# rgcgithub/regenie

Hardware: NVIDIA H100
Metric: step1_level0_snps_per_sec (higher is better)
Workload: dtype int8 Gram + int8 prediction (both exact integer sums) + tf32x3 factorisation + f64 refinement / statistics

## Files before the change

regenie_b200/csrc/bed_kernels.cu:

```cuda
#include "kernels.cuh"

namespace rg {

__device__ __forceinline__ uint32_t plink_to_code(uint32_t v, int ref_first) {
  const uint32_t lut = ref_first ? 0x9Cu : 0x1Eu;
  return (lut >> (2 * v)) & 3u;
}

__global__ void bed_relayout_kernel(const uint8_t* __restrict__ packed, int64_t row_stride, int bs,
                                    const int32_t* __restrict__ file_idx_pad, const int32_t* __restrict__ word_base,
                                    const uint32_t* __restrict__ word_keep, int ref_first,
                                    uint32_t* __restrict__ gp, int64_t words_per_row) {
  const int64_t w = blockIdx.x * (int64_t)blockDim.x + threadIdx.x;
  const int row = blockIdx.y;
  if (w >= words_per_row) return;
  uint32_t out = 0;
  const int base = (row < bs) ? __ldg(word_base + w) : -1;
  if (base >= 0) {
    const uint8_t* p = packed + (int64_t)row * row_stride + (base >> 2);
    const int64_t left = row_stride - (base >> 2);
    uint64_t x = 0;
#pragma unroll
    for (int b = 0; b < 5; ++b)
      if (b < left) x |= (uint64_t)__ldg(p + b) << (8 * b);
    const uint32_t v = (uint32_t)(x >> (2 * (base & 3)));
    const uint32_t H = (v >> 1) & 0x55555555u, Lo = v & 0x55555555u;
    const uint32_t oh = ref_first ? Lo : (~H & 0x55555555u);
    out = ((oh << 1) | (H ^ Lo)) & __ldg(word_keep + w);
  } else if (base == -2) {
    const uint8_t* prow = packed + (int64_t)row * row_stride;
    const int4* fi4 = reinterpret_cast<const int4*>(file_idx_pad + w * 16);
#pragma unroll
    for (int q = 0; q < 4; ++q) {
      const int4 f = __ldg(fi4 + q);
      const int fi[4] = {f.x, f.y, f.z, f.w};
#pragma unroll
      for (int k = 0; k < 4; ++k) {
        uint32_t code = 0;
        if (fi[k] >= 0) {
          const uint32_t b = __ldg(prow + (fi[k] >> 2));
          code = plink_to_code((b >> (2 * (fi[k] & 3))) & 3u, ref_first);
        }
        out |= code << (2 * (q * 4 + k));
      }
    }
  }
  gp[(int64_t)row * words_per_row + w] = out;
}

__device__ __forceinline__ uint32_t spread_sel(uint32_t b) {
  return (b & 0x3u) | ((b & 0xCu) << 2) | ((b & 0x30u) << 4) | ((b & 0xC0u) << 6);
}

__global__ void bed_expand_fp8_kernel(const uint32_t* __restrict__ gp, int64_t words_per_row,
                                      int rows_p, uint8_t* __restrict__ z, int64_t npad) {
  const int64_t w = blockIdx.x * (int64_t)blockDim.x + threadIdx.x;
  const int row = blockIdx.y;
  if (w >= words_per_row) return;
  const uint32_t word = __ldg(gp + (int64_t)row * words_per_row + w);
  const uint32_t kLutG = 0x00100800u;
  const uint32_t kLutM = 0x08000000u;
  uint4 g, m;
  uint32_t* gv = reinterpret_cast<uint32_t*>(&g);
  uint32_t* mv = reinterpret_cast<uint32_t*>(&m);
#pragma unroll
  for (int k = 0; k < 4; ++k) {
    const uint32_t sel = spread_sel((word >> (8 * k)) & 0xFFu);
    gv[k] = __byte_perm(kLutG, 0, sel);
    mv[k] = __byte_perm(kLutM, 0, sel);
  }
  *reinterpret_cast<uint4*>(z + (int64_t)row * npad + w * 16) = g;
  *reinterpret_cast<uint4*>(z + (int64_t)(rows_p + row) * npad + w * 16) = m;
}

void launch_bed_relayout(const uint8_t* packed, int64_t row_stride, int bs, int rows_p,
                         const int32_t* file_idx_pad, const int32_t* word_base, const uint32_t* word_keep, int ref_first,
                         uint32_t* gp, int64_t npad,
                         cudaStream_t s) {
  const int64_t wpr = npad / 16;
  dim3 grid((unsigned)ceil_div(wpr, 256), rows_p);
  bed_relayout_kernel<<<grid, 256, 0, s>>>(packed, row_stride, bs, file_idx_pad, word_base, word_keep, ref_first, gp, wpr);
}

void launch_bed_expand_fp8(const uint32_t* gp, int rows_p, uint8_t* z, int64_t npad, cudaStream_t s) {
  const int64_t wpr = npad / 16;
  dim3 grid((unsigned)ceil_div(wpr, 256), rows_p);
  bed_expand_fp8_kernel<<<grid, 256, 0, s>>>(gp, wpr, rows_p, z, npad);
}

}
```

regenie_b200/csrc/context.cuh:

```cuda
#pragma once
#include <map>
#include <memory>

#include "../../include/rg_b200.h"
#include "kernels.cuh"

struct rg_ctx;
namespace rg { void ensure_W(::rg_ctx* h); }

struct rg_ctx {
  int kind = 0;
  int device = 0;
  cudaStream_t stream = nullptr;
  int64_t launches = 0;

  int64_t N = 0, Npad = 0, n_analyzed = 0;
  int C = 0, P = 0, K = 1, R = 0, R1 = 0, loocv = 0;
  int bs_max = 0, rows_p_max = 0, total_blocks = 0, cpp = 0;
  int64_t B = 0;

  std::vector<int64_t> fold_sizes, fold_pad_start, fold_pad_len;
  std::vector<int32_t> pad_of;
  std::vector<int32_t> src_of;
  std::vector<uint8_t> in_analysis;
  std::vector<int32_t> cached_sample_idx;
  bool file_idx_valid = false;
  int nchunks = 0;

  rg::DevBuf<double> xy;
  rg::DevBuf<uint8_t> mask;
  rg::DevBuf<uint8_t> is_real;
  rg::DevBuf<int32_t> tile_fold;
  rg::DevBuf<int4> chunks;
  rg::DevBuf<int2> fold_chunks;
  rg::DevBuf<int2> fold_k;
  rg::DevBuf<double> XtX_f, XtY_f, lambda, neff;
  rg::DevBuf<int32_t> file_idx_pad;
  rg::DevBuf<int32_t> word_base;
  rg::DevBuf<uint32_t> word_keep;
  rg::DevBuf<unsigned long long> err_slot;
  cudaStream_t poll_stream = nullptr;
  unsigned long long* poll_host = nullptr;

  struct Lane {
    cudaStream_t stream = nullptr;
    cudaEvent_t done = nullptr;
    cudaEvent_t h2d_done = nullptr;
    bool h2d_recorded = false;
    rg::DevBuf<uint8_t> packed_dev;
    rg::DevBuf<uint8_t> packed_buf[2];
    cudaStream_t copy_stream = nullptr;
    cudaEvent_t relayout_done[2] = {nullptr, nullptr};
    bool relayout_recorded[2] = {false, false};
    int packed_flip = 0;
    rg::DevBuf<uint8_t> pgen_in;
    rg::DevBuf<uint32_t> gp;
    rg::DevBuf<uint8_t> z;
    rg::DevBuf<float> zz;
    rg::DevBuf<unsigned long long> miss_total;
    rg::DevBuf<int2> miss_seg;
    rg::DevBuf<int32_t> miss_list;
    rg::DevBuf<uint32_t> gt;
    rg::DevBuf<float> tstat;
    rg::DevBuf<int32_t> cnt_part, cnt_fold;
    rg::DevBuf<double> sum_part, sum_fold;
    rg::DevBuf<double> mu, inv_sd, Bv, Af, Qf, gty_f, rhs;
    rg::DevBuf<double> cm;
    rg::DevBuf<double> inv;
    rg::DevBuf<double> gam, gmu, cvec, part, mean_invsd;
    std::map<int, CUtensorMap> tmaps;
    rg::DevBuf<uint8_t> dig;
    rg::DevBuf<double> wraw;
    rg::DevBuf<double*> wraw_tab;
    rg::DevBuf<double> dscale;
    std::map<int, CUtensorMap> dmaps;
    std::map<int, CUtensorMap> gmaps;
    rg::DevBuf<uint8_t> dense_in;
    rg::DevBuf<double> gd, dpart, dpart_y;
    std::unique_ptr<rg::MixedSolver> mx;
    rg::DevBuf<double> mx_Af, mx_b, mx_x, mx_r;
    rg::DevBuf<unsigned int> mx_fail;
    unsigned int* mx_fail_host = nullptr;
    cudaEvent_t mx_ev = nullptr;
    bool mx_pending = false;
    int mx_bs = 0, mx_block_id = 0;
    int last_pred_i8 = 0, last_mx_n = 0;
    bool last_gram_dense = false;
  };
  std::vector<std::unique_ptr<Lane>> lanes;
  int next_lane = 0, last_lane = 0;
  rg::DevBuf<uint8_t> packed_dev;
  rg::DevBuf<uint32_t> gp;
  struct TileList {
    rg::DevBuf<int2> buf;
    int count = 0;
  };
  std::map<int, TileList> tile_lists, stat_tile_lists;
  bool stats_tc = false;
  int stat_drows = 0;
  rg::DevBuf<uint8_t> xyD;
  rg::DevBuf<double> xy_scale;
  CUtensorMap tmD;

  rg::DevBuf<double> W;
  int last_bs = 0, last_rows_p = 0, last_nC = 0, last_n_aug = 0, last_nmat = 0;

  rg::DevBuf<int4> l1_chunks;
  rg::DevBuf<int2> l1_fold_chunks;
  int l1_nchunks = 0;
  rg::DevBuf<double> l1_part, l1_part_y, l1_cm, l1_inv, l1_beta, l1_sums, l1_part_out, l1_tau, l1_pred;
  rg::DevBuf<int32_t> l1_chr_cols;
  rg::DevBuf<double> l1_zrows, l1_hvec, l1_bvec;
  std::vector<int32_t> best_idx;
  std::vector<double> prs_host;
  int l1_nC = 0;
  int l1_nmat = 0, l1_n_aug = 0;
  int64_t l1_chunk_len = 0;
  bool l1_done = false;
  rg::DevBuf<double*> W_tab;
  std::vector<double*> W_host_tab;
  std::vector<uint8_t> W_owned;
  std::vector<void*> W_peer_mapped;
  std::vector<uint8_t> l1_select;
  bool l1_bt = false;
  rg::DevBuf<double> lg_Ws, lg_eta, lg_p, lg_wm, lg_res, lg_off, lg_beta, lg_score, lg_q, lg_devp, lg_scal;
  rg::DevBuf<int8_t> lg_ym;
  rg::DevBuf<int2> lg_all_chunks;

  int strict = 0, dp = 0;
  std::vector<double> Xh;
  std::vector<uint8_t> maskh;
  rg::DevBuf<double> F, s2_part, s2_sums, s2_maskcount, s2_YtX, s2_XmX, s2_scf;
  rg::DevBuf<double> s2_out_d;
  rg::DevBuf<int32_t> s2_out_i;
  double* s2_hd = nullptr;
  int32_t* s2_hi = nullptr;
  size_t s2_host_cap = 0;
  bool s2_tc = false;
  int s2_drows = 0, s2_nchunk = 0, s2_ncol = 0;
  int64_t s2_chunk_len = 0;
  rg::DevBuf<uint8_t> s2_z3, s2_FD;
  rg::DevBuf<double> s2_Fscale;
  rg::DevBuf<float> s2_T;
  rg::DevBuf<int2> s2_fold_k;
  std::map<int, std::unique_ptr<rg::DevBuf<int2>>> s2_tile_lists;
  rg::DevBuf<uint8_t> s2_ones;
  CUtensorMap s2_tmD;
  std::map<int, CUtensorMap> s2_tmZ;
  std::map<int, int> s2_ntiles;
  std::vector<uint8_t> s2_male;
  int s2_col_male = -1, bt_col_male = -1;
  rg::DevBuf<uint8_t> s2_nonpar;
  bool s2_nonpar_set = false;
  rg::DevBuf<double> s2_male_tot;
  int bt_mode = 0, bt_dp = 0, bt_ncol = 0;
  int s2_fcols = 0;
  bool s2_chr_set = false, bt_chr_set = false;
  int s2_last_bs = 0;
  int s2_sums_rows = 0, bt_sums_rows = 0, bt_sums_dp = 0;
  static constexpr int kStageSlots = 4;
  rg::DevBuf<uint8_t> s2_stage[kStageSlots];
  cudaStream_t s2_copy_stream = nullptr;
  cudaEvent_t s2_stage_ev[kStageSlots] = {nullptr, nullptr, nullptr, nullptr};
  bool s2_stage_pending[kStageSlots] = {false, false, false, false};
  rg::DevBuf<uint8_t> probs_dev, miss_dev;
  rg::DevBuf<uint8_t> inflate_comp, inflate_raw;
  rg::DevBuf<uint64_t> inflate_offs;
  rg::DevBuf<int32_t> inflate_status;
  rg::DevBuf<uint8_t> pgen_in, pgen_rows;
  rg::DevBuf<unsigned long long> pgen_err;
  rg::DevBuf<uint32_t> dz;
  rg::DevBuf<double> bt_F, bt_w, bt_gs, bt_xw, bt_off, bt_coltot, bt_xwy, bt_part, bt_sums, bt_nnz, bt_n510;
  rg::DevBuf<double> bt_xtwg, bt_mu, bt_info, firth_gvec, firth_out, bt_den, bt_phat;
  rg::DevBuf<int8_t> bt_ym, firth_cflag;
  rg::DevBuf<int2> bt_cnt_part;
  rg::DevBuf<int32_t> firth_sel, firth_status;

  bool gram_dense = false;
  int64_t miss_cap = 0;

  int solver_mixed = 1;
  float mx_tol = 1e-9f;
  int64_t mx_blocks = 0, mx_fallbacks = 0;

  bool timing = false;
  cudaEvent_t ev0 = nullptr, ev1 = nullptr;
  std::map<std::string, std::pair<double, int64_t>> timers;
  std::vector<std::tuple<std::string, cudaEvent_t, cudaEvent_t>> pending;
};

namespace rg {
void require_gpu(int device);
void ensure_file_idx(rg_ctx* h, const int32_t* sample_idx);
void flush_timers(rg_ctx* h);
void sync_lanes(rg_ctx* h);
void pgen_check_errors(rg_ctx* h);
}

#define RG_API_BEGIN try {
#define RG_API_END                         \
  }                                        \
  catch (const rg::Error& e) {             \
    rg::set_last_error(e.msg);             \
    return 1;                              \
  }                                        \
  catch (const std::exception& e) {        \
    rg::set_last_error(e.what());          \
    return 1;                              \
  }                                        \
  return 0;
```

regenie_b200/csrc/gram_wgmma.cu:

```cuda
#include "kernels.cuh"
#include "wgmma_sm90.cuh"

namespace rg {

namespace {

using namespace sm90;

constexpr int BM = 128;
constexpr int BK = 128;
constexpr int STAGES = 4;
constexpr int A_BYTES = BM * BK;
constexpr int NTHREADS = 288;

}

template <int BN>
__global__ void __launch_bounds__(NTHREADS, 1)
gram_s8_wgmma_kernel(const __grid_constant__ CUtensorMap tmZ, const __grid_constant__ CUtensorMap tmB,
                      const int2* __restrict__ tiles,
                      const int2* __restrict__ fold_k, float* __restrict__ out, int ldo,
                      int64_t fold_stride, float out_scale, const unsigned long long* __restrict__ miss_total,
                      unsigned long long miss_cap, int miss_tile0) {
  constexpr int B_BYTES = BN * BK;
  constexpr int STAGE_BYTES = A_BYTES + B_BYTES;
  constexpr int NACC = BN / 2;
  extern __shared__ uint8_t smem_raw[];
  const uint32_t raw = smem_u32(smem_raw);
  const uint32_t base = (raw + 1023u) & ~1023u;
  uint8_t* gen_base = smem_raw + (base - raw);
  const uint32_t sA = base;
  const uint32_t sB = base + STAGES * A_BYTES;
  uint64_t* bars = reinterpret_cast<uint64_t*>(gen_base + STAGES * STAGE_BYTES);
  const uint32_t full_bar = smem_u32(bars);
  const uint32_t empty_bar = smem_u32(bars + STAGES);

  const int warp = __shfl_sync(0xffffffffu, threadIdx.x >> 5, 0), lane = threadIdx.x & 31;
  const int2 tile = tiles[blockIdx.x];
  if (miss_total && tile.x >= miss_tile0 && *miss_total <= miss_cap) return;
  const int2 fk = fold_k[blockIdx.y];
  const int nkb = fk.y;

  if (warp == 8 && lane == 0) {
    for (int s = 0; s < STAGES; ++s) {
      mbar_init(full_bar + 8 * s, 1);
      mbar_init(empty_bar + 8 * s, 2);
    }
    fence_barrier_init();
    prefetch_tmap(&tmZ);
    prefetch_tmap(&tmB);
  }
  __syncthreads();

  if (warp == 8) {
    if (lane == 0) {
      for (int kb = 0; kb < nkb; ++kb) {
        const int s = kb % STAGES;
        const uint32_t ph = (kb / STAGES) & 1;
        mbar_wait(empty_bar + 8 * s, ph ^ 1);
        mbar_expect_tx(full_bar + 8 * s, STAGE_BYTES);
        const int kc = (fk.x + kb) * BK;
        tma_load_2d(sA + s * A_BYTES, &tmZ, full_bar + 8 * s, kc, tile.x * BM);
        tma_load_2d(sB + s * B_BYTES, &tmB, full_bar + 8 * s, kc, tile.y * BN);
        if (BN == 256) tma_load_2d(sB + s * B_BYTES + A_BYTES, &tmB, full_bar + 8 * s, kc, tile.y * BN + 128);
      }
    }
    return;
  }

  const int wg = warp >> 2;
  int32_t acc[NACC];
#pragma unroll
  for (int i = 0; i < NACC; ++i) acc[i] = 0;
  fence_regs(acc);
  for (int kb = 0; kb < nkb; ++kb) {
    const int s = kb % STAGES;
    const uint32_t ph = (kb / STAGES) & 1;
    mbar_wait(full_bar + 8 * s, ph);
    const uint64_t da = desc_k128(sA + s * A_BYTES + wg * (64 * BK));
    const uint64_t db = desc_k128(sB + s * B_BYTES);
    wgmma_fence();
#pragma unroll
    for (int k = 0; k < BK / 32; ++k) {
      if constexpr (BN == 256) wgmma_s8_n256(acc, da + (uint64_t)(2 * k), db + (uint64_t)(2 * k));
      else wgmma_s8_n128(acc, da + (uint64_t)(2 * k), db + (uint64_t)(2 * k));
    }
    wgmma_commit();
    wgmma_wait<1>();
    if (kb > 0 && (warp & 3) == 0 && lane == 0) mbar_arrive(empty_bar + 8 * ((kb - 1) % STAGES));
  }
  wgmma_wait<0>();
  fence_regs(acc);

  const int r0 = tile.x * BM + wg * 64 + (warp & 3) * 16 + (lane >> 2);
  float* obase = out + (int64_t)blockIdx.y * fold_stride + tile.y * BN + 2 * (lane & 3);
#pragma unroll
  for (int j = 0; j < BN / 8; ++j) {
    *reinterpret_cast<float2*>(obase + (int64_t)r0 * ldo + 8 * j) =
        make_float2((float)acc[4 * j] * out_scale, (float)acc[4 * j + 1] * out_scale);
    *reinterpret_cast<float2*>(obase + (int64_t)(r0 + 8) * ldo + 8 * j) =
        make_float2((float)acc[4 * j + 2] * out_scale, (float)acc[4 * j + 3] * out_scale);
  }
}

__global__ void gram_reference_kernel(const uint8_t* __restrict__ z, int64_t npad, int rows2, int k0, int k1,
                                      float* __restrict__ out, int ldo) {
  const int j = blockIdx.x * blockDim.x + threadIdx.x;
  const int i = blockIdx.y;
  if (j >= rows2 || j > i) return;
  const uint8_t* zi = z + (int64_t)i * npad;
  const uint8_t* zj = z + (int64_t)j * npad;
  int acc = 0;
  for (int t = k0; t < k1; ++t) {
    const int a = zi[t] >> 3;
    const int b = zj[t] >> 3;
    acc += a * b;
  }
  out[(int64_t)i * ldo + j] = (float)acc;
}

typedef CUresult (*EncodeTiledFn)(CUtensorMap*, CUtensorMapDataType, cuuint32_t, void*, const cuuint64_t*,
                                  const cuuint64_t*, const cuuint32_t*, const cuuint32_t*, CUtensorMapInterleave,
                                  CUtensorMapSwizzle, CUtensorMapL2promotion, CUtensorMapFloatOOBfill);

static EncodeTiledFn get_encode_fn() {
  static EncodeTiledFn fn = nullptr;
  if (!fn) {
    void* p = nullptr;
    cudaDriverEntryPointQueryResult qres;
    RG_CUDA(cudaGetDriverEntryPoint("cuTensorMapEncodeTiled", &p, cudaEnableDefault, &qres));
    RG_CHECK(p != nullptr && qres == cudaDriverEntryPointSuccess, "cuTensorMapEncodeTiled not available");
    fn = reinterpret_cast<EncodeTiledFn>(p);
  }
  return fn;
}

void make_gram_tensor_map(CUtensorMap* tm, const uint8_t* z, int64_t npad, int rows2) {
  const cuuint64_t gdim[2] = {(cuuint64_t)npad, (cuuint64_t)rows2};
  const cuuint64_t gstride[1] = {(cuuint64_t)npad};
  const cuuint32_t box[2] = {BK, 128};
  const cuuint32_t estr[2] = {1, 1};
  CUresult r = get_encode_fn()(tm, CU_TENSOR_MAP_DATA_TYPE_UINT8, 2, const_cast<uint8_t*>(z), gdim, gstride, box,
                               estr, CU_TENSOR_MAP_INTERLEAVE_NONE, CU_TENSOR_MAP_SWIZZLE_128B,
                               CU_TENSOR_MAP_L2_PROMOTION_L2_256B, CU_TENSOR_MAP_FLOAT_OOB_FILL_NONE);
  RG_CHECK(r == CUDA_SUCCESS, "cuTensorMapEncodeTiled failed (" + std::to_string((int)r) + ")");
}

size_t gram_smem_bytes(int bn) {
  return (size_t)STAGES * (A_BYTES + bn * BK) + 1024 + 128;
}

void gram_tile_list(int rows2, std::vector<int2>& tiles) {
  tiles.clear();
  for (int nj = 0; nj < rows2 / 256; ++nj)
    for (int mi = 2 * nj; mi < rows2 / BM; ++mi) tiles.push_back(make_int2(mi, nj));
}

void launch_gram_wgmma(const CUtensorMap& tm, const CUtensorMap& tmB, const int2* tiles, int ntiles, const int2* fold_k, int K,
                         float* out, int ldo, int64_t fold_stride, float out_scale, cudaStream_t s, int bn,
                         const unsigned long long* miss_total, int64_t miss_cap, int miss_tile0) {
  RG_CHECK(bn == 256 || bn == 128, "gram tiles are 128 x 256 or 128 x 128");
  dim3 grid(ntiles, K);
  if (bn == 256) {
    ensure_dyn_smem(reinterpret_cast<const void*>(gram_s8_wgmma_kernel<256>), gram_smem_bytes(256));
    gram_s8_wgmma_kernel<256><<<grid, NTHREADS, gram_smem_bytes(256), s>>>(tm, tmB, tiles, fold_k, out, ldo, fold_stride, out_scale,
                                                                                     miss_total, miss_cap, miss_tile0);
  } else {
    ensure_dyn_smem(reinterpret_cast<const void*>(gram_s8_wgmma_kernel<128>), gram_smem_bytes(128));
    gram_s8_wgmma_kernel<128><<<grid, NTHREADS, gram_smem_bytes(128), s>>>(tm, tmB, tiles, fold_k, out, ldo, fold_stride, out_scale,
                                                                                     miss_total, miss_cap, miss_tile0);
  }
}

void launch_gram_reference(const uint8_t* z, int64_t npad, int rows2, int k0, int k1, float* out, int ldo,
                           cudaStream_t s) {
  dim3 grid((unsigned)ceil_div(rows2, 128), rows2);
  gram_reference_kernel<<<grid, 128, 0, s>>>(z, npad, rows2, k0, k1, out, ldo);
}

}
```

regenie_b200/csrc/kernels.cuh:

```cuda
#pragma once
#include "common.cuh"

namespace rg {

constexpr int kMaxFolds = 16;
constexpr int kMaxCov = 64;
constexpr int kMaxRidge = 8;
constexpr int kMaxPhenoTile = 8;
constexpr int kLimbs = 9;
constexpr int kLimbsI8 = 5;
constexpr int kLimbQI8 = 50;

void launch_bed_relayout(const uint8_t* packed, int64_t row_stride, int bs, int rows_p,
                         const int32_t* file_idx_pad, const int32_t* word_base, const uint32_t* word_keep, int ref_first,
                         uint32_t* gp, int64_t npad,
                         cudaStream_t s);
void launch_bed_expand_fp8(const uint32_t* gp, int rows_p, uint8_t* z, int64_t npad, cudaStream_t s);

struct SnpFinalizeArgs {
  int bs, rows_p, C, P, K, cpp, loocv;
  long long n_analyzed;
  double numtol;
  const int32_t* cnt_fold;
  const double* sum_fold;
  const double* XtX_f;
  const double* XtY_f;
  double *mu, *inv_sd;
  double* Bv;
  double *Af, *Qf;
  double *gty_f, *rhs;
  unsigned long long* err_slot;
  long long err_base;
};

struct AssembleArgs {
  int bs, rows_p, nC, C, K, R, loocv;
  const float* zz;
  int64_t ldz, zz_fold_stride;
  const double *mu, *inv_sd, *Bv, *Af, *Qf;
  const double* lambda;
  double* cm;
  int64_t cm_stride;
  int ldc;
  float* planes = nullptr;
  float* lplanes = nullptr;
};

void launch_l0_stats(const uint32_t* gp, int64_t npad, const double* xy, int cpp, const int4* chunks,
                     int nchunks, int rows_p, int32_t* cnt_part, double* sum_part, cudaStream_t s);
void launch_l0_fold_reduce(const int32_t* cnt_part, const double* sum_part, int rows_p, int cpp,
                           const int2* fold_chunks, int K, int32_t* cnt_fold, double* sum_fold,
                           cudaStream_t s);
void launch_l0_snp_finalize(const SnpFinalizeArgs& a, cudaStream_t s);
void launch_l0_assemble(const AssembleArgs& a, const double* rhs, int P, int Ppad, int nmat, cudaStream_t s);

void make_gram_tensor_map(CUtensorMap* tm, const uint8_t* z, int64_t npad, int rows2);
size_t gram_smem_bytes(int bn = 256);
constexpr int kStatQ = 14;
constexpr int kStatOnesRow = 126;
void launch_l0_xy_digits(const double* xy, int cpp, int ncol, int64_t npad, const uint8_t* is_real, double* scale,
                         uint8_t* D, cudaStream_t s);
void launch_l0_stats_finish(const float* T, int ldt, int64_t t_fold_stride, const float* zz, int ldz,
                            int64_t zz_fold_stride, int rows_p, int cpp, int ncol, int K, const double* scale,
                            int32_t* cnt_fold, double* sum_fold, cudaStream_t s);
void gram_tile_list(int rows2, std::vector<int2>& tiles);
void launch_gram_wgmma(const CUtensorMap& tm, const CUtensorMap& tmB, const int2* tiles, int ntiles, const int2* fold_k, int K,
                         float* out, int ldo, int64_t fold_stride, float out_scale, cudaStream_t s, int bn = 256,
                         const unsigned long long* miss_total = nullptr, int64_t miss_cap = 0, int miss_tile0 = 0);
constexpr float kZScaleGram = 1.f / 64;
constexpr float kZScaleStat = 1.f / 8;
constexpr double kMissSparseRate = 0.015;
void launch_miss_list(const uint32_t* gp, int64_t npad, int rows_p, const int2* fold_k, int K, unsigned long long* total,
                      int64_t cap, int2* seg, int32_t* list, cudaStream_t s);
void launch_miss_transpose(const uint32_t* gp, int64_t npad, int rows_p, const unsigned long long* total, int64_t cap,
                           uint32_t* gt, cudaStream_t s);
void launch_miss_sparse(const uint32_t* gt, int rows_p, const int2* seg, const int32_t* list, int K,
                        const unsigned long long* total, int64_t cap, float* zz, int64_t fold_stride, cudaStream_t s);
void launch_gram_reference(const uint8_t* z, int64_t npad, int rows2, int k0, int k1, float* out, int ldo,
                           cudaStream_t s);

void launch_chol_factor(double* cm, int64_t stride, int nC, int n_aug, int batch, double* inv,
                        unsigned long long* err_slot, long long err_base, cudaStream_t s);
void launch_chol_backsolve(double* cm, int64_t stride, int nC, int P, int batch, const double* inv,
                           cudaStream_t s);
int chol_num_launches(int nC);
size_t chol_inv_elems(int nC, int batch);
void launch_chol_rows_backsolve(double* cm, int64_t stride, int nC, int row0, int nrows, int batch,
                                const double* inv, cudaStream_t s);

struct Tf32GemmEpilogue {
  int n;
  int64_t out_mat_stride;
  float* out;
  int mirror;
  int b_cols_local;
  int negate;
  int lower_only;
  const double* cin;
  int64_t cin_mat_stride;
  int cin_ld, cin_mat_div;
  const double* diag_add;
  int diag_mod;
  int c_chunks;
  int c_mat_div;
};
void make_tf32_operand_tensor_map(CUtensorMap* tm, const float* base, int cols, int rows, int batch);
void make_f32_rows_tensor_map(CUtensorMap* tm, const float* base, int cols, int64_t rows, int box_cols, int box_rows);
void launch_tf32x3_gemm(const CUtensorMap& tmA, const CUtensorMap& tmB, const int4* tiles, int ntiles, int batch,
                        const Tf32GemmEpilogue& ep, cudaStream_t s, const CUtensorMap* tmC = nullptr);

constexpr int kMxMaxSteps = 6;
class MixedSolver {
 public:
  MixedSolver();
  ~MixedSolver();
  MixedSolver(const MixedSolver&) = delete;
  MixedSolver& operator=(const MixedSolver&) = delete;
  static int dim_for(int bs);
  void prepare(int n, int K, int R, int Pp);
  float* a_planes();
  float* l_planes();
  void solve(const double* Af, const double* lambda, const double* bvec, double* xvec, double* rvec, int P, int steps,
             float tol, unsigned int* fail_flag, cudaStream_t s, bool first_col_ready = false);
  static int launches_per_solve(int n, int steps, int P);
  const float* debug_planes(int which) const;
 private:
  struct Impl;
  Impl* impl;
};
void launch_l0_assemble_sym(const AssembleArgs& a, const double* rhs, int P, int Pp, double* bvec, cudaStream_t s);

void launch_dense_from_dosage(const uint8_t* probs, const uint8_t* miss, int64_t n_file, int bs, const int32_t* file_idx_pad,
                              int ref_first, double* gd, int64_t npad, cudaStream_t s);
void launch_dense_from_f64(const double* G, int64_t n_file, int bs, const int32_t* file_idx_pad, double* gd, int64_t npad,
                           cudaStream_t s);
void launch_dense_prepare(double* gd, int64_t npad, int bs, const int32_t* file_idx_pad, const double* xy, int cpp, int C,
                          long long n_analyzed, double numtol, double* mu, double* sd, unsigned long long* err_slot,
                          long long err_base, cudaStream_t s);
void launch_dense_assemble(const double* part, int64_t part_stride, int ldp, const double* part_y, int64_t part_y_stride,
                           const int2* fold_chunks, int K, int R, const double* lambda, int bs, int nC, int P, double* cm,
                           int64_t cm_stride, int loocv, cudaStream_t s);
void launch_dense_loocv_fill(const double* gd, int64_t npad, int bs, int nC, double* cm, int64_t cm_stride, int row0, int R,
                             cudaStream_t s);
void launch_dense_predict(const double* gd, int64_t npad, int bs, const double* cm, int64_t cm_stride, int ldc, int nC, int R,
                          int P, const int32_t* tile_fold, const uint8_t* mask, double* const* W, int col0, cudaStream_t s);

struct PredictArgs {
  int bs, rows_p, C, P, R, Qp, cpp, col0;
  int64_t npad, words_per_row;
  const uint32_t* gp;
  const int32_t* tile_fold;
  const double *gam, *gmu;
  const double* cvec;
  const double* xy;
  const uint8_t* mask;
  double* const* W;
  double* part;
};
void launch_l0_gamma(const double* cm, int64_t cm_stride, int ldc, int nC, int R, int P, int Qp,
                     int bs, int rows_p, int K, const double* mu, const double* inv_sd,
                     const double* Bv, int C, double* gam, double* gmu, double* cvec, cudaStream_t s);
void launch_l0_predict(const PredictArgs& a, int ntiles, cudaStream_t s);
void launch_l0_standardize(const double* part, int ntiles, int Qp, int Q, int P, const double* neff,
                           double* mean_invsd, double* const* W, int64_t npad, int col0,
                           const uint8_t* is_real, cudaStream_t s, const double* const* src = nullptr, int src_col0 = 0);
int predict_qt();

struct PredictTcArgs {
  int rows_p, C, P, Q, Qp, cpp, col0, ngroups;
  int64_t npad;
  const int32_t* tile_fold;
  const double* scale;
  const double* cvec;
  const double* xy;
  const uint8_t* mask;
  double* const* W;
  double* part;
};
void make_byte_tensor_map(CUtensorMap* tm, const uint8_t* basep, int64_t inner, int64_t rows);
void make_gp_tensor_map(CUtensorMap* tm, const uint32_t* gp, int64_t words_per_row, int64_t rows);
int launch_l0_colsum(double* const* W, int64_t npad, int col0, int P, int Q, int Qp, double* part,
                     cudaStream_t s);
size_t predict_i8_dig_bytes(int K, int ngroups, int rows_p);
void launch_l0_coef_i8(const double* cm, int64_t cm_stride, int ldc, int nC, int R, int P, int Q, int Qp, int bs,
                       int rows_p, int K, const double* mu, const double* inv_sd, const double* Bv, int C, double* gam,
                       double* gmu, double* cvec, double* scale, uint8_t* dig, int ngroups, cudaStream_t s);
void launch_l0_predict_i8(const CUtensorMap& tmG, const CUtensorMap& tmD, const PredictTcArgs& a, int ntiles,
                          cudaStream_t s);

void launch_l1_gram(const double* W, int64_t ldw, int B, const int4* chunks, int nchunks, double* part,
                    int64_t part_stride, int ldp, cudaStream_t s);
void launch_l1_xty(const double* W, int64_t ldw, const double* xy, int cpp, int ycol, const int4* chunks,
                   int nchunks, double* part_y, int B, cudaStream_t s);
void launch_l1_assemble(const double* part, int64_t part_stride, int ldp, const double* part_y,
                        const int2* fold_chunks, int K, int R1, const double* tau, int B, int nC, double* cm,
                        int64_t cm_stride, int loocv, cudaStream_t s);
void launch_l1_pred_sums(const double* W, int64_t ldw, int B, int R1, const double* beta, int ldb,
                         const int32_t* tile_fold, const double* xy, int cpp, int ycol, double* part_out,
                         int ntiles, double* out, cudaStream_t s);
void launch_l1_chr_pred(const double* W, int64_t ldw, int nchr, const int32_t* chr_col_start, const double* beta,
                        int ldb, int R1, int best, const int32_t* tile_fold, double* pred, int64_t npad,
                        cudaStream_t s);

void launch_l0_loocv_fill(const uint32_t* gp, int64_t npad, int bs, int nC, const double* mu, const double* inv_sd,
                          const double* Bv, int C, const double* xy, int cpp, double* cm, int64_t cm_stride,
                          int nrow0, int R, cudaStream_t s);
void launch_l0_loocv_pred(const double* cm, int64_t cm_stride, int nC, int bs, int Ppad, int P, int R,
                          const double* xy, int cpp, int C, const uint8_t* mask, int64_t npad, double* const* W,
                          int col0, double* part, int Qp, cudaStream_t s);
void launch_l0_loocv_std_apply(double* const* W, int64_t npad, int col0, int P, int Q, const uint8_t* mask,
                               const double* mean_invsd, cudaStream_t s);
void launch_l1_loocv_fill(const double* W, int64_t ldw, int B, int nC, double* cm, int64_t cm_stride, int nrow0,
                          int R1, int64_t npad, cudaStream_t s);
void launch_l1_loocv_sums(const double* cm, int64_t cm_stride, int nC, int B, int nrow0, const double* xy, int cpp,
                          int ycol, double* part, int R1, int ntiles, double* out, cudaStream_t s);
void launch_rows_sqnorm(const double* rows, int nC, int B, double* out, int ntiles, cudaStream_t s);

void launch_l1_scale_rows(const double* W, int64_t ldw, int B, const double* wm, double* Ws, cudaStream_t s);
void launch_l1_bt_eta(const double* W, int64_t ldw, int B, const double* beta, const double* offset, const int8_t* ym,
                      double* eta, double* pv, double* wm, double* resid, double* dev_part, double* dev_out,
                      cudaStream_t s);
void launch_l1_bt_score(const double* part_y, int nchunks, int B, int nC, double tau, const double* beta, double* score,
                        double* rhs_row, cudaStream_t s);
void launch_l1_bt_loo_sums(const double* eta, const double* q, const double* wm, const double* resid, const int8_t* ym,
                           double eps, double* fvec, double* part, double* out6, int64_t npad, cudaStream_t s);
void launch_l1_bt_chr_pred(const double* W, int64_t ldw, int nC, const double* zrows, const double* fvec,
                           const double* bvec, int nchr, const int32_t* chr_col_start, double* pred, int64_t npad,
                           cudaStream_t s);
void launch_l1_loocv_chr_pred(const double* W, int64_t ldw, int B, int nC, const double* zrows, const double* hvec,
                              const double* bvec, const double* xy, int cpp, int ycol, int nchr,
                              const int32_t* chr_col_start, double* pred, int64_t npad, cudaStream_t s);
void launch_l0_std_reduce_only(const double* part, int ntiles, int Qp, int Q, int P, const double* neff,
                               double* mean_invsd, cudaStream_t s);

struct S2FinalizeArgs {
  int bs, C, P, dp, strict;
  long long n_analyzed, n_samples;
  double min_mac, numtol;
  const double* sums;
  const double* mask_count;
  const double* YtX;
  const double* XmX;
  const double* scf_sv;
  const uint8_t* non_par = nullptr;
  int col_male = -1;
  const double* male_tot = nullptr;
  const double* nz_count = nullptr;
  const double* info_sums = nullptr;
  double* info = nullptr;
  double *af, *mac, *af_all, *mac_all, *scale_fac, *stat, *beta, *se, *chisq;
  int32_t *ns, *ns_all, *flags;
};
void launch_s2_stats(const uint32_t* gp, int64_t npad, const double* F, int dp, const int4* chunks, int nchunks,
                     int rows_p, double* part, double* sums, cudaStream_t s);
void launch_s2_finalize(const S2FinalizeArgs& a, cudaStream_t s);
void launch_bed_expand3_fp8(const uint32_t* gp, int rows_p, uint8_t* z, int64_t npad, cudaStream_t s);
void launch_s2_bt_bed_finish(const float* T, int ldt, int64_t chunk_stride, int nchunk, int rows_p, int dp, int D,
                             const double* scale, double* sums4, double* nnz, double* n2, cudaStream_t s);
void launch_gp_to_dz(const uint32_t* gp, int rows_p, uint32_t* dz, int64_t npad, cudaStream_t s);
void launch_s2_stats_finish(const float* T, int ldt, int64_t chunk_stride, int nchunk, int rows_p, int dp, int D,
                            const double* scale, double* sums, cudaStream_t s);

struct S2BtFinalizeArgs {
  int bs, C, P, dp, with_flip;
  long long n_analyzed, n_samples;
  double min_mac, numtol;
  const double* sums;
  const double* col_tot;
  const double* xwy;
  const uint8_t* non_par = nullptr;
  int col_male = -1;
  double unit = 255.0;
  const double* nz_count;
  const double* n510;
  double *af, *mac, *info, *af_all, *mac_all, *scale_fac, *stat, *beta, *se, *chisq, *xtwg, *mu, *den;
  int32_t *ns, *ns_all, *flags;
};
void launch_dosage_relayout(const uint8_t* probs, const uint8_t* miss, int64_t n_file, int bs, int rows_p,
                            const int32_t* file_idx_pad, int ref_first, uint32_t* dz, int64_t npad, cudaStream_t s);
void launch_dosage_stats(const uint32_t* dz, int64_t npad, const double* F, int dp, const int4* chunks, int nchunks,
                         int rows_p, double* part, int2* part_cnt, double* sums, double* nnz, double* n510, cudaStream_t s,
                         int ncol = 0 );
void launch_s2_bt_finalize(const S2BtFinalizeArgs& a, cudaStream_t s);
void launch_dosage_scale(const double* sums4, int rows_p, int dp, double* sums3, double* se, cudaStream_t s);

struct FirthArgs {
  int n_sel, C, P, dp, niter;
  double tol, maxstep;
  int64_t npad;
  const int32_t *sel_var, *sel_trait;
  const uint32_t* dz;
  const double* F;
  const double *w, *gs, *xw, *off;
  const int8_t* ym;
  const double* xtwg;
  const double* mu;
  const double* mac;
  const int32_t* flags;
  double* gvec;
  int8_t* cflag;
  double *beta, *se, *lrt;
  int32_t* status;
};
void launch_s2_firth(const FirthArgs& a, cudaStream_t s);

struct SpaArgs {
  int n_sel, C, P, dp, niter;
  double tol;
  int64_t npad;
  const int32_t *sel_var, *sel_trait;
  const uint32_t* dz;
  const double* F;
  const double *w, *gs, *xw, *phat;
  const int8_t* ym;
  const double* xtwg;
  const double* mu;
  const double *stat, *den;
  const int32_t* flags;
  double* gvec;
  int8_t* cflag;
  double* pval;
  int32_t* status;
};
void launch_s2_spa(const SpaArgs& a, cudaStream_t s);

}
```

regenie_b200/csrc/rg_api.cu:

```cuda
#include <string.h>

#include <algorithm>
#include <mutex>

#include "context.cuh"

namespace rg {

static thread_local std::string g_last_error;
void set_last_error(const std::string& m) { g_last_error = m; }

bool is_device_pointer(const void* p) {
  cudaPointerAttributes at;
  cudaError_t e = cudaPointerGetAttributes(&at, p);
  if (e != cudaSuccess) {
    cudaGetLastError();
    return false;
  }
  return at.type == cudaMemoryTypeDevice || at.type == cudaMemoryTypeManaged;
}

void copy_to_device(void* dst, const void* src, size_t bytes, cudaStream_t stream) {
  if (bytes == 0) return;
  RG_CUDA(cudaMemcpyAsync(dst, src, bytes, cudaMemcpyDefault, stream));
}

struct ScopedTimer {
  rg_ctx* h;
  std::string name;
  cudaEvent_t a = nullptr, b = nullptr;
  cudaStream_t st;
  ScopedTimer(rg_ctx* h_, const char* n, cudaStream_t s_) : h(h_), name(n), st(s_) {
    if (!h->timing) return;
    cudaEventCreate(&a);
    cudaEventCreate(&b);
    cudaEventRecord(a, st);
  }
  ~ScopedTimer() {
    if (!h->timing) return;
    cudaEventRecord(b, st);
    h->pending.emplace_back(name, a, b);
  }
};

void flush_timers(rg_ctx* h) {
  for (auto& t : h->pending) {
    float ms = 0.f;
    cudaEventSynchronize(std::get<2>(t));
    cudaEventElapsedTime(&ms, std::get<1>(t), std::get<2>(t));
    auto& acc = h->timers[std::get<0>(t)];
    acc.first += ms;
    acc.second += 1;
    cudaEventDestroy(std::get<1>(t));
    cudaEventDestroy(std::get<2>(t));
  }
  h->pending.clear();
}

void require_gpu(int device) {
  int n = 0;
  cudaError_t e = cudaGetDeviceCount(&n);
  if (e != cudaSuccess || n == 0) {
    cudaGetLastError();
    throw Error{"no CUDA device available: librg_b200 has no CPU fallback"};
  }
  RG_CHECK(device >= 0 && device < n, "invalid CUDA device ordinal");
  cudaDeviceProp prop;
  RG_CUDA(cudaGetDeviceProperties(&prop, device));
  RG_CHECK(prop.major == 9 && prop.minor == 0, std::string("librg_b200 is built for sm_90a only; device is sm_") +
                                 std::to_string(prop.major) + std::to_string(prop.minor));
}

static void build_layout(rg_ctx* h, const double* X, const double* Y, const uint8_t* mask,
                         const uint8_t* in_analysis, const int64_t* fold_sizes) {
  const int64_t N = h->N;
  const int K = h->K, C = h->C, P = h->P;
  h->fold_sizes.assign(K, 0);
  if (h->loocv) {
    h->fold_sizes[0] = N;
  } else {
    int64_t tot = 0;
    for (int f = 0; f < K; ++f) {
      RG_CHECK(fold_sizes[f] > 0, "fold sizes must be positive");
      h->fold_sizes[f] = fold_sizes[f];
      tot += fold_sizes[f];
    }
    RG_CHECK(tot == N, "fold sizes must sum to n_samples");
  }
  h->fold_pad_start.assign(K, 0);
  h->fold_pad_len.assign(K, 0);
  int64_t off = 0;
  for (int f = 0; f < K; ++f) {
    h->fold_pad_start[f] = off;
    h->fold_pad_len[f] = round_up(h->fold_sizes[f], kFoldPad);
    off += h->fold_pad_len[f];
  }
  h->Npad = off;
  RG_CHECK(h->Npad < (1ll << 31), "padded sample count must fit in int32");
  h->pad_of.assign(N, 0);
  h->src_of.assign(h->Npad, -1);
  std::vector<int32_t> tile_fold(h->Npad / 128);
  {
    int64_t s = 0;
    for (int f = 0; f < K; ++f) {
      for (int64_t o = 0; o < h->fold_sizes[f]; ++o, ++s) {
        h->pad_of[s] = (int32_t)(h->fold_pad_start[f] + o);
        h->src_of[h->fold_pad_start[f] + o] = (int32_t)s;
      }
      for (int64_t t = h->fold_pad_start[f]; t < h->fold_pad_start[f] + h->fold_pad_len[f]; t += 128)
        tile_fold[t / 128] = f;
    }
  }
  h->in_analysis.assign(in_analysis, in_analysis + N);

  h->cpp = (int)round_up(C + P, 16);
  std::vector<double> xy((size_t)h->Npad * h->cpp, 0.0);
  std::vector<uint8_t> maskp((size_t)P * h->Npad, 0), is_real(h->Npad, 0);
  h->maskh.assign(mask, mask + (size_t)N * P);
  for (int64_t s = 0; s < N; ++s) {
    const int64_t t = h->pad_of[s];
    is_real[t] = 1;
    double* r = &xy[(size_t)t * h->cpp];
    for (int c = 0; c < C; ++c) r[c] = X[(size_t)c * N + s];
    for (int p = 0; p < P; ++p) {
      r[C + p] = Y[(size_t)p * N + s];
      maskp[(size_t)p * h->Npad + t] = mask[(size_t)p * N + s] ? 1 : 0;
    }
  }
  std::vector<double> XtX((size_t)K * C * C, 0.0), XtY((size_t)K * C * P, 0.0);
  {
    std::vector<double> cXtX(XtX.size(), 0.0), cXtY(XtY.size(), 0.0);
    auto add = [](double& sum, double& comp, double v) {
      const double t = sum + v;
      comp += (std::fabs(sum) >= std::fabs(v)) ? (sum - t) + v : (v - t) + sum;
      sum = t;
    };
    int64_t s = 0;
    for (int f = 0; f < K; ++f)
      for (int64_t o = 0; o < h->fold_sizes[f]; ++o, ++s)
        for (int c = 0; c < C; ++c) {
          const double xc = X[(size_t)c * N + s];
          if (xc == 0.0) continue;
          for (int c2 = 0; c2 < C; ++c2) {
            const size_t e = ((size_t)f * C + c) * C + c2;
            add(XtX[e], cXtX[e], xc * X[(size_t)c2 * N + s]);
          }
          for (int p = 0; p < P; ++p) {
            const size_t e = ((size_t)f * C + c) * P + p;
            add(XtY[e], cXtY[e], xc * Y[(size_t)p * N + s]);
          }
        }
    for (size_t e = 0; e < XtX.size(); ++e) XtX[e] += cXtX[e];
    for (size_t e = 0; e < XtY.size(); ++e) XtY[e] += cXtY[e];
  }
  std::vector<int4> chunks;
  std::vector<int2> fold_chunks(K), fold_k(K);
  for (int f = 0; f < K; ++f) {
    fold_chunks[f].x = (int)chunks.size();
    for (int64_t o = 0; o < h->fold_pad_len[f]; o += kStatChunk) {
      const int len = (int)std::min<int64_t>(kStatChunk, h->fold_pad_len[f] - o);
      chunks.push_back(make_int4((int)(h->fold_pad_start[f] + o), len, f, 0));
    }
    fold_chunks[f].y = (int)chunks.size();
    fold_k[f] = make_int2((int)(h->fold_pad_start[f] / 128), (int)(h->fold_pad_len[f] / 128));
  }
  h->nchunks = (int)chunks.size();

  cudaStream_t s = h->stream;
  h->xy.alloc(xy.size());
  h->mask.alloc(maskp.size());
  h->is_real.alloc(is_real.size());
  h->tile_fold.alloc(tile_fold.size());
  h->chunks.alloc(chunks.size());
  h->fold_chunks.alloc(K);
  h->fold_k.alloc(K);
  h->XtX_f.alloc(XtX.size());
  h->XtY_f.alloc(XtY.size());
  RG_CUDA(cudaMemcpyAsync(h->xy.p, xy.data(), xy.size() * 8, cudaMemcpyHostToDevice, s));
  RG_CUDA(cudaMemcpyAsync(h->mask.p, maskp.data(), maskp.size(), cudaMemcpyHostToDevice, s));
  RG_CUDA(cudaMemcpyAsync(h->is_real.p, is_real.data(), is_real.size(), cudaMemcpyHostToDevice, s));
  RG_CUDA(cudaMemcpyAsync(h->tile_fold.p, tile_fold.data(), tile_fold.size() * 4, cudaMemcpyHostToDevice, s));
  RG_CUDA(cudaMemcpyAsync(h->chunks.p, chunks.data(), chunks.size() * sizeof(int4), cudaMemcpyHostToDevice, s));
  RG_CUDA(cudaMemcpyAsync(h->fold_chunks.p, fold_chunks.data(), K * sizeof(int2), cudaMemcpyHostToDevice, s));
  RG_CUDA(cudaMemcpyAsync(h->fold_k.p, fold_k.data(), K * sizeof(int2), cudaMemcpyHostToDevice, s));
  RG_CUDA(cudaMemcpyAsync(h->XtX_f.p, XtX.data(), XtX.size() * 8, cudaMemcpyHostToDevice, s));
  RG_CUDA(cudaMemcpyAsync(h->XtY_f.p, XtY.data(), XtY.size() * 8, cudaMemcpyHostToDevice, s));
  {
    int64_t max_fold = 0;
    for (int f = 0; f < K; ++f) max_fold = std::max(max_fold, h->fold_pad_len[f]);
    const char* e = getenv("RG_B200_STATS");
    h->stats_tc = !(e && std::string(e) == "f64") && max_fold * 30 < (1ll << 24);
    if (h->stats_tc) {
      const int ngroups = (int)ceil_div(C + P, kStatQ);
      h->stat_drows = ngroups * 128;
      h->xyD.alloc((size_t)h->stat_drows * h->Npad);
      h->xy_scale.alloc(h->cpp);
      RG_CUDA(cudaMemsetAsync(h->xyD.p, 0, (size_t)h->stat_drows * h->Npad, s));
      launch_l0_xy_digits(h->xy.p, h->cpp, C + P, h->Npad, h->is_real.p, h->xy_scale.p, h->xyD.p, s);
      make_gram_tensor_map(&h->tmD, h->xyD.p, h->Npad, h->stat_drows);
    }
  }
  {
    const char* e = getenv("RG_B200_GRAM");
    const std::string mode = e ? e : "";
    h->gram_dense = mode == "dense";
    const double rate = mode == "sparse" ? 1.0 : kMissSparseRate;
    h->miss_cap = std::min<int64_t>((int64_t)(rate * h->bs_max * h->n_analyzed), INT32_MAX);
  }
  RG_CUDA(cudaStreamSynchronize(s));
}

static void build_file_idx(rg_ctx* h, const int32_t* sample_idx_host) {
  std::vector<int32_t> fi(h->Npad, -1);
  for (int64_t t = 0; t < h->Npad; ++t) {
    const int32_t s = h->src_of[t];
    if (s < 0 || !h->in_analysis[s]) continue;
    fi[t] = sample_idx_host ? sample_idx_host[s] : s;
  }
  const int64_t nw = h->Npad / 16;
  std::vector<int32_t> wb(nw, -1);
  std::vector<uint32_t> wk(nw, 0);
  for (int64_t w = 0; w < nw; ++w) {
    int32_t base = -1;
    bool contiguous = true;
    for (int j = 0; j < 16; ++j) {
      const int32_t f = fi[w * 16 + j];
      if (f < 0) continue;
      wk[w] |= 3u << (2 * j);
      if (base == -1) base = f - j;
      else if (f - j != base) contiguous = false;
    }
    wb[w] = (wk[w] == 0) ? -1 : ((contiguous && base >= 0) ? base : -2);
  }
  h->file_idx_pad.alloc(h->Npad);
  h->word_base.alloc(nw);
  h->word_keep.alloc(nw);
  RG_CUDA(cudaMemcpyAsync(h->word_base.p, wb.data(), nw * 4, cudaMemcpyHostToDevice, h->stream));
  RG_CUDA(cudaMemcpyAsync(h->word_keep.p, wk.data(), nw * 4, cudaMemcpyHostToDevice, h->stream));
  RG_CUDA(cudaMemcpyAsync(h->file_idx_pad.p, fi.data(), fi.size() * 4, cudaMemcpyHostToDevice, h->stream));
  RG_CUDA(cudaStreamSynchronize(h->stream));
  h->file_idx_valid = true;
}

void ensure_file_idx(rg_ctx* h, const int32_t* sample_idx) {
  if (!sample_idx) {
    if (!h->file_idx_valid || !h->cached_sample_idx.empty()) {
      build_file_idx(h, nullptr);
      h->cached_sample_idx.clear();
    }
    return;
  }
  std::vector<int32_t> host_idx(h->N);
  if (is_device_pointer(sample_idx)) RG_CUDA(cudaMemcpy(host_idx.data(), sample_idx, h->N * 4, cudaMemcpyDefault));
  else host_idx.assign(sample_idx, sample_idx + h->N);
  if (!h->file_idx_valid || h->cached_sample_idx != host_idx) {
    build_file_idx(h, host_idx.data());
    h->cached_sample_idx = std::move(host_idx);
  }
}

void ensure_W(::rg_ctx* h) {
  if (h->W.p) return;
  size_t n_owned = 0;
  for (int p = 0; p < h->P; ++p) n_owned += h->W_owned[p] ? 1 : 0;
  const size_t per = (size_t)h->Npad * h->B;
  h->W.alloc(std::max<size_t>(1, n_owned) * per);
  RG_CUDA(cudaMemset(h->W.p, 0, std::max<size_t>(1, n_owned) * per * 8));
  size_t slot = 0;
  for (int p = 0; p < h->P; ++p)
    if (h->W_owned[p]) h->W_host_tab[p] = h->W.p + (slot++) * per;
  RG_CUDA(cudaMemcpy(h->W_tab.p, h->W_host_tab.data(), h->P * sizeof(double*), cudaMemcpyHostToDevice));
}

struct BlockDims {
  int bs, rows_p, nC, Ppad, n_aug, nmat, Q, Qp, col0, block_id, ntiles_s;
};

static int mx_pp(int P) { return (int)round_up(P, 2); }
constexpr int kMxSteps = 3;

static AssembleArgs assemble_args(const rg_ctx* h, const rg_ctx::Lane& L, const BlockDims& d) {
  AssembleArgs aa;
  aa.bs = d.bs; aa.rows_p = d.rows_p; aa.C = h->C; aa.K = h->K; aa.R = h->R; aa.loocv = h->loocv;
  aa.zz = L.zz.p; aa.ldz = 2 * d.rows_p; aa.zz_fold_stride = (int64_t)4 * d.rows_p * d.rows_p;
  aa.mu = L.mu.p; aa.inv_sd = L.inv_sd.p; aa.Bv = L.Bv.p; aa.Af = L.Af.p; aa.Qf = L.Qf.p;
  aa.lambda = h->lambda.p;
  return aa;
}

static void ensure_f64_systems(rg_ctx* h, rg_ctx::Lane& L, const BlockDims& d, cudaStream_t s) {
  const int nC_max = (int)round_up(h->bs_max, 64);
  const size_t need = (size_t)d.nmat * (nC_max + d.Ppad + (h->loocv ? h->Npad : 0)) * nC_max;
  if (L.cm.n < need) {
    L.cm.alloc(need);
    RG_CUDA(cudaMemsetAsync(L.cm.p, 0, need * 8, s));
  }
  L.inv.alloc(chol_inv_elems(nC_max, d.nmat));
}

static void enqueue_loocv_predict(rg_ctx* h, rg_ctx::Lane& L, const BlockDims& d, cudaStream_t s) {
  const int P = h->P;
  launch_l0_loocv_pred(L.cm.p, (int64_t)d.n_aug * d.nC, d.nC, d.bs, d.Ppad, P, h->R, h->xy.p, h->cpp, h->C, h->mask.p, h->Npad,
                       h->W_tab.p, d.col0, L.part.p, d.Qp, s);
  launch_l0_std_reduce_only(L.part.p, d.ntiles_s, d.Qp, d.Q, P, h->neff.p, L.mean_invsd.p, s);
  launch_l0_loocv_std_apply(h->W_tab.p, h->Npad, d.col0, P, d.Q, h->mask.p, L.mean_invsd.p, s);
  h->launches += 3;
}

static void enqueue_solve_f64(rg_ctx* h, rg_ctx::Lane& L, const BlockDims& d, cudaStream_t s) {
  const int C = h->C, P = h->P, R = h->R;
  ensure_f64_systems(h, L, d, s);
  AssembleArgs aa = assemble_args(h, L, d);
  aa.nC = d.nC; aa.cm = L.cm.p; aa.cm_stride = (int64_t)d.n_aug * d.nC; aa.ldc = d.nC;
  {
    ScopedTimer t(h, "l0_assemble", s);
    launch_l0_assemble(aa, L.rhs.p, P, d.Ppad, d.nmat, s);
    h->launches += 2;
  }
  if (h->loocv) {
    ScopedTimer t(h, "loocv_fill", s);
    launch_l0_loocv_fill(L.gp.p, h->Npad, d.bs, d.nC, L.mu.p, L.inv_sd.p, L.Bv.p, C, h->xy.p, h->cpp, L.cm.p, aa.cm_stride,
                         d.nC + d.Ppad, R, s);
    h->launches += 1;
  }
  {
    ScopedTimer t(h, "chol_factor", s);
    launch_chol_factor(L.cm.p, aa.cm_stride, d.nC, d.n_aug, d.nmat, L.inv.p, h->err_slot.p,
                       (long long)(1ll << 40) + (long long)d.block_id * 1024, s);
    h->launches += chol_num_launches(d.nC);
  }
  if (h->loocv) {
    ScopedTimer t(h, "l0_predict", s);
    enqueue_loocv_predict(h, L, d, s);
    return;
  }
  {
    ScopedTimer t(h, "chol_backsolve", s);
    launch_chol_backsolve(L.cm.p, aa.cm_stride, d.nC, P, d.nmat, L.inv.p, s);
    h->launches += 1;
  }
}

static void enqueue_solve_mixed(rg_ctx* h, rg_ctx::Lane& L, const BlockDims& d, int n, cudaStream_t s) {
  const int P = h->P, K = h->K, R = h->R;
  const int Pp = mx_pp(P);
  if (!L.mx) {
    L.mx = std::make_unique<MixedSolver>();
    L.mx_fail.alloc(1);
    RG_CUDA(cudaMallocHost(&L.mx_fail_host, sizeof(unsigned int)));
    RG_CUDA(cudaEventCreateWithFlags(&L.mx_ev, cudaEventDisableTiming));
  }
  const size_t need_A = (size_t)K * n * n, need_b = (size_t)K * Pp * n, need_x = (size_t)K * R * Pp * n;
  L.mx_Af.alloc(need_A);
  L.mx_b.alloc(need_b);
  L.mx_x.alloc(need_x);
  L.mx_r.alloc(need_x);
  RG_CHECK(L.mx_Af.n >= need_A && L.mx_b.n >= need_b && L.mx_x.n >= need_x && L.mx_r.n >= need_x,
           "mixed solver: scratch smaller than the block's systems");
  L.mx->prepare(n, K, R, Pp);
  RG_CUDA(cudaMemsetAsync(L.mx_fail.p, 0, sizeof(unsigned int), s));
  AssembleArgs aa = assemble_args(h, L, d);
  aa.nC = n; aa.cm = L.mx_Af.p; aa.cm_stride = (int64_t)n * n; aa.ldc = n;
  aa.planes = L.mx->a_planes();
  aa.lplanes = L.mx->l_planes();
  {
    ScopedTimer t(h, "l0_assemble", s);
    launch_l0_assemble_sym(aa, L.rhs.p, P, Pp, L.mx_b.p, s);
    h->launches += 2;
  }
  {
    ScopedTimer t(h, "mx_solve", s);
    L.mx->solve(L.mx_Af.p, h->lambda.p, L.mx_b.p, L.mx_x.p, L.mx_r.p, P, kMxSteps, h->mx_tol, L.mx_fail.p, s, true);
    h->launches += MixedSolver::launches_per_solve(n, kMxSteps, P) - 1;
  }
}

static void enqueue_predict(rg_ctx* h, rg_ctx::Lane& L, const BlockDims& d, const double* xsrc, int64_t xstride, int xld,
                            int xrow0, cudaStream_t s) {
  const int C = h->C, P = h->P, K = h->K, R = h->R;
  const int64_t Npad = h->Npad;
  ScopedTimer t(h, "l0_predict", s);
  if (L.wraw.n < (size_t)P * R * Npad) {
    L.wraw.alloc((size_t)P * R * Npad);
    L.wraw_tab.alloc(P);
    std::vector<double*> tab(P);
    for (int p = 0; p < P; ++p) tab[p] = L.wraw.p + (size_t)p * R * Npad;
    RG_CUDA(cudaMemcpyAsync(L.wraw_tab.p, tab.data(), P * sizeof(double*), cudaMemcpyHostToDevice, s));
    RG_CUDA(cudaStreamSynchronize(s));
  }
  PredictArgs pa;
  pa.bs = d.bs; pa.rows_p = d.rows_p; pa.C = C; pa.P = P; pa.R = R; pa.Qp = d.Qp; pa.cpp = h->cpp;
  pa.col0 = 0; pa.npad = Npad; pa.words_per_row = Npad / 16;
  pa.gp = L.gp.p; pa.tile_fold = h->tile_fold.p; pa.gam = L.gam.p; pa.gmu = L.gmu.p;
  pa.cvec = L.cvec.p; pa.xy = h->xy.p; pa.mask = h->mask.p; pa.W = L.wraw_tab.p; pa.part = L.part.p;
  const bool use_i8 = 2 * d.rows_p <= 4096;
  L.last_pred_i8 = use_i8 ? 1 : 0;
  if (!use_i8) {
    launch_l0_gamma(xsrc, xstride, xld, xrow0, R, P, d.Qp, d.bs, d.rows_p, K, L.mu.p, L.inv_sd.p, L.Bv.p, C,
                    L.gam.p, L.gmu.p, L.cvec.p, s);
    launch_l0_predict(pa, d.ntiles_s, s);
    h->launches += 3;
  } else {
    const int ngroups = (int)ceil_div(d.Q, kLimbQI8);
    const int drows_per_group = 256;
    const size_t need = predict_i8_dig_bytes(K, ngroups, h->rows_p_max);
    if (L.dig.n < need) {
      L.dig.alloc(need);
      RG_CUDA(cudaMemsetAsync(L.dig.p, 0, need, s));
      L.dmaps.clear();
    }
    L.dscale.alloc((size_t)K * d.Qp);
    if (!L.dmaps.count(d.rows_p)) {
      CUtensorMap tm;
      make_byte_tensor_map(&tm, L.dig.p, 2 * d.rows_p, (int64_t)K * ngroups * drows_per_group);
      L.dmaps[d.rows_p] = tm;
    }
    if (!L.gmaps.count(d.rows_p)) {
      CUtensorMap tm;
      make_gp_tensor_map(&tm, L.gp.p, Npad / 16, d.rows_p);
      L.gmaps[d.rows_p] = tm;
    }
    launch_l0_coef_i8(xsrc, xstride, xld, xrow0, R, P, d.Q, d.Qp, d.bs, d.rows_p, K, L.mu.p, L.inv_sd.p, L.Bv.p, C,
                      L.gam.p, L.gmu.p, L.cvec.p, L.dscale.p, L.dig.p, ngroups, s);
    PredictTcArgs ta;
    ta.rows_p = d.rows_p; ta.C = C; ta.P = P; ta.Q = d.Q; ta.Qp = d.Qp; ta.cpp = h->cpp; ta.col0 = 0; ta.ngroups = ngroups;
    ta.npad = Npad; ta.tile_fold = h->tile_fold.p; ta.scale = L.dscale.p; ta.cvec = L.cvec.p;
    ta.xy = h->xy.p; ta.mask = h->mask.p; ta.W = L.wraw_tab.p; ta.part = L.part.p;
    launch_l0_predict_i8(L.gmaps[d.rows_p], L.dmaps[d.rows_p], ta, d.ntiles_s, s);
    h->launches += 2;
  }
  launch_l0_standardize(L.part.p, d.ntiles_s, d.Qp, d.Q, P, h->neff.p, L.mean_invsd.p, h->W_tab.p, Npad, d.col0,
                        h->is_real.p, s, L.wraw_tab.p, 0);
  h->launches += 2;
}

static BlockDims block_dims(const rg_ctx* h, int bs, int block_id) {
  BlockDims d;
  d.bs = bs; d.rows_p = (int)round_up(bs, kRowPad); d.nC = (int)round_up(bs, 64); d.Ppad = (int)round_up(h->P, 64);
  d.n_aug = d.nC + d.Ppad + (h->loocv ? (int)h->Npad : 0);
  d.nmat = (h->loocv ? 1 : h->K) * h->R;
  d.Q = h->R * h->P; d.Qp = (int)round_up(d.Q, predict_qt());
  d.col0 = block_id * h->R; d.block_id = block_id; d.ntiles_s = (int)(h->Npad / 128);
  return d;
}

void resolve_lane(rg_ctx* h, rg_ctx::Lane& L) {
  if (!L.mx_pending) return;
  RG_CUDA(cudaEventSynchronize(L.mx_ev));
  L.mx_pending = false;
  if (*L.mx_fail_host == 0) return;
  h->mx_fallbacks += 1;
  L.last_mx_n = 0;
  const BlockDims d = block_dims(h, L.mx_bs, L.mx_block_id);
  enqueue_solve_f64(h, L, d, L.stream);
  enqueue_predict(h, L, d, L.cm.p, (int64_t)d.n_aug * d.nC, d.nC, d.nC, L.stream);
}

void sync_lanes(rg_ctx* h) {
  RG_CUDA(cudaSetDevice(h->device));
  for (auto& l : h->lanes) resolve_lane(h, *l);
  for (auto& l : h->lanes) RG_CUDA(cudaStreamSynchronize(l->stream));
}

static rg_ctx::Lane& l0_begin_block(rg_ctx* h, int bs, int block_id, const int32_t* sample_idx, BlockDims& d) {
  RG_CHECK(h->kind == 1, "handle is not a Step-1 handle");
  RG_CHECK(bs > 0 && bs <= h->bs_max, "block size out of range");
  RG_CHECK(block_id >= 0 && block_id < h->total_blocks, "block_id out of range");
  ensure_W(h);
  for (int p = 0; p < h->P; ++p)
    RG_CHECK(h->W_host_tab[p] != nullptr, "a phenotype has neither local storage nor an attached owner (rg_W_set_owned / rg_W_attach_peer)");
  RG_CUDA(cudaSetDevice(h->device));
  ensure_file_idx(h, sample_idx);
  rg_ctx::Lane& L = *h->lanes[h->next_lane];
  h->last_lane = h->next_lane;
  h->next_lane = (h->next_lane + 1) % (int)h->lanes.size();
  d = block_dims(h, bs, block_id);
  h->last_bs = bs; h->last_rows_p = d.rows_p; h->last_nC = d.nC; h->last_n_aug = d.n_aug; h->last_nmat = d.nmat;
  return L;
}

template <class Fill>
static const rg_ctx::TileList& cached_tiles(std::map<int, rg_ctx::TileList>& cache, int rows_p, Fill fill) {
  rg_ctx::TileList& e = cache[rows_p];
  if (e.count == 0) {
    std::vector<int2> tiles;
    fill(tiles);
    e.buf.alloc(tiles.size());
    RG_CUDA(cudaMemcpy(e.buf.p, tiles.data(), tiles.size() * sizeof(int2), cudaMemcpyHostToDevice));
    e.count = (int)tiles.size();
  }
  return e;
}

static void l0_block_bed(rg_ctx* h, const uint8_t* packed, int64_t row_stride, int bs,
                         const int32_t* sample_idx, int ref_first, int block_id) {
  BlockDims d;
  rg_ctx::Lane& L = l0_begin_block(h, bs, block_id, sample_idx, d);
  const int C = h->C, P = h->P, K = h->K;
  const int rows_p = d.rows_p, Qp = d.Qp;
  const int64_t Npad = h->Npad;
  cudaStream_t s = L.stream;

  const uint8_t* packed_d = packed;
  int staged = -1;
  if (!is_device_pointer(packed)) {
    staged = (L.packed_flip ^= 1);
    rg::DevBuf<uint8_t>& buf = L.packed_buf[staged];
    buf.alloc((size_t)h->bs_max * row_stride);
    if (!L.copy_stream) RG_CUDA(cudaStreamCreateWithFlags(&L.copy_stream, cudaStreamNonBlocking));
    if (!L.h2d_done) RG_CUDA(cudaEventCreateWithFlags(&L.h2d_done, cudaEventDisableTiming));
    cudaStream_t cs = L.copy_stream;
    if (L.relayout_recorded[staged]) RG_CUDA(cudaStreamWaitEvent(cs, L.relayout_done[staged], 0));
    {
      ScopedTimer t(h, "h2d", cs);
      copy_to_device(buf.p, packed, (size_t)bs * row_stride, cs);
    }
    RG_CUDA(cudaEventRecord(L.h2d_done, cs));
    L.h2d_recorded = true;
    RG_CUDA(cudaStreamWaitEvent(s, L.h2d_done, 0));
    packed_d = buf.p;
  }
  resolve_lane(h, L);

  L.gp.alloc((size_t)h->rows_p_max * (Npad / 16));
  L.z.alloc((size_t)2 * h->rows_p_max * Npad);
  L.zz.alloc((size_t)K * 4 * h->rows_p_max * h->rows_p_max);
  L.cnt_part.alloc((size_t)h->nchunks * h->rows_p_max * 4);
  L.sum_part.alloc((size_t)h->nchunks * h->rows_p_max * 2 * h->cpp);
  L.cnt_fold.alloc((size_t)K * h->rows_p_max * 4);
  L.sum_fold.alloc((size_t)K * h->rows_p_max * 2 * h->cpp);
  L.mu.alloc(h->rows_p_max);
  L.inv_sd.alloc(h->rows_p_max);
  L.Bv.alloc((size_t)h->rows_p_max * C);
  L.Af.alloc((size_t)K * h->rows_p_max * C);
  L.Qf.alloc((size_t)K * h->rows_p_max * C);
  L.gty_f.alloc((size_t)K * h->rows_p_max * P);
  L.rhs.alloc((size_t)K * h->rows_p_max * P);
  const int Kg = h->loocv ? 1 : K;
  L.gam.alloc((size_t)Kg * h->rows_p_max * Qp);
  L.gmu.alloc((size_t)Kg * h->rows_p_max * Qp);
  L.cvec.alloc((size_t)Kg * Qp * C);
  L.part.alloc((size_t)d.ntiles_s * Qp * 2);
  L.mean_invsd.alloc((size_t)2 * Qp);

  {
    ScopedTimer t(h, "bed_relayout", s);
    launch_bed_relayout(packed_d, row_stride, bs, rows_p, h->file_idx_pad.p, h->word_base.p, h->word_keep.p, ref_first, L.gp.p, Npad, s);
    if (staged >= 0) {
      if (!L.relayout_done[staged]) RG_CUDA(cudaEventCreateWithFlags(&L.relayout_done[staged], cudaEventDisableTiming));
      RG_CUDA(cudaEventRecord(L.relayout_done[staged], s));
      L.relayout_recorded[staged] = true;
    }
  }
  {
    ScopedTimer t(h, "bed_expand", s);
    launch_bed_expand_fp8(L.gp.p, rows_p, L.z.p, Npad, s);
  }
  h->launches += 2;

  auto snp_finalize = [&]() {
    SnpFinalizeArgs a;
    a.bs = bs; a.rows_p = rows_p; a.C = C; a.P = P; a.K = K; a.cpp = h->cpp; a.loocv = h->loocv;
    a.n_analyzed = h->n_analyzed; a.numtol = 1e-6;
    a.cnt_fold = L.cnt_fold.p; a.sum_fold = L.sum_fold.p; a.XtX_f = h->XtX_f.p; a.XtY_f = h->XtY_f.p;
    a.mu = L.mu.p; a.inv_sd = L.inv_sd.p; a.Bv = L.Bv.p; a.Af = L.Af.p; a.Qf = L.Qf.p;
    a.gty_f = L.gty_f.p; a.rhs = L.rhs.p; a.err_slot = h->err_slot.p;
    a.err_base = (long long)block_id * h->bs_max;
    launch_l0_snp_finalize(a, s);
    h->launches += 1;
  };
  if (!h->stats_tc) {
    ScopedTimer t(h, "l0_stats", s);
    launch_l0_stats(L.gp.p, Npad, h->xy.p, h->cpp, h->chunks.p, h->nchunks, rows_p, L.cnt_part.p,
                    L.sum_part.p, s);
    launch_l0_fold_reduce(L.cnt_part.p, L.sum_part.p, rows_p, h->cpp, h->fold_chunks.p, K,
                          L.cnt_fold.p, L.sum_fold.p, s);
    snp_finalize();
    h->launches += 2;
  }

  {
    if (!L.tmaps.count(rows_p)) {
      CUtensorMap tm;
      make_gram_tensor_map(&tm, L.z.p, Npad, 2 * rows_p);
      L.tmaps[rows_p] = tm;
    }
    const rg_ctx::TileList& tl =
        cached_tiles(h->tile_lists, rows_p, [&](std::vector<int2>& tiles) { gram_tile_list(2 * rows_p, tiles); });
    const int64_t zz_stride = (int64_t)4 * rows_p * rows_p;
    ScopedTimer t(h, "gram_wgmma", s);
    if (h->gram_dense) {
      launch_gram_wgmma(L.tmaps[rows_p], L.tmaps[rows_p], tl.buf.p, tl.count, h->fold_k.p, K,
                        L.zz.p, 2 * rows_p, zz_stride, kZScaleGram, s);
      h->launches += 1;
    } else {
      L.miss_total.alloc(1);
      L.miss_seg.alloc((size_t)K * h->rows_p_max);
      L.miss_list.alloc((size_t)std::max<int64_t>(h->miss_cap, 1));
      L.gt.alloc((size_t)Npad * (h->rows_p_max / 16));
      launch_miss_list(L.gp.p, Npad, rows_p, h->fold_k.p, K, L.miss_total.p, h->miss_cap, L.miss_seg.p, L.miss_list.p, s);
      launch_miss_transpose(L.gp.p, Npad, rows_p, L.miss_total.p, h->miss_cap, L.gt.p, s);
      launch_gram_wgmma(L.tmaps[rows_p], L.tmaps[rows_p], tl.buf.p, tl.count, h->fold_k.p, K,
                        L.zz.p, 2 * rows_p, zz_stride, kZScaleGram, s, 256, L.miss_total.p, h->miss_cap, rows_p / 128);
      launch_miss_sparse(L.gt.p, rows_p, L.miss_seg.p, L.miss_list.p, K, L.miss_total.p, h->miss_cap, L.zz.p, zz_stride, s);
      h->launches += 5;
    }
    L.last_gram_dense = h->gram_dense;
  }
  if (h->stats_tc) {
    ScopedTimer t(h, "l0_stats", s);
    const int stat_bn = (h->stat_drows % 256 == 0) ? 256 : 128;
    const rg_ctx::TileList& tl = cached_tiles(h->stat_tile_lists, rows_p, [&](std::vector<int2>& tiles) {
      for (int nj = 0; nj < h->stat_drows / stat_bn; ++nj)
        for (int mi = 0; mi < 2 * rows_p / 128; ++mi) tiles.push_back(make_int2(mi, nj));
    });
    L.tstat.alloc((size_t)K * 2 * h->rows_p_max * h->stat_drows);
    const int64_t tfs = (int64_t)2 * rows_p * h->stat_drows;
    launch_gram_wgmma(L.tmaps[rows_p], h->tmD, tl.buf.p, tl.count, h->fold_k.p,
                      K, L.tstat.p, h->stat_drows, tfs, kZScaleStat, s, stat_bn);
    launch_l0_stats_finish(L.tstat.p, h->stat_drows, tfs, L.zz.p, 2 * rows_p, (int64_t)4 * rows_p * rows_p, rows_p,
                           h->cpp, C + P, K, h->xy_scale.p, L.cnt_fold.p, L.sum_fold.p, s);
    snp_finalize();
    h->launches += 2;
  }

  const int mx_n = (!h->loocv && h->solver_mixed) ? MixedSolver::dim_for(bs) : 0;
  L.last_mx_n = mx_n;
  if (mx_n > 0) {
    enqueue_solve_mixed(h, L, d, mx_n, s);
    enqueue_predict(h, L, d, L.mx_x.p, (int64_t)mx_pp(P) * mx_n, mx_n, 0, s);
    RG_CUDA(cudaMemcpyAsync(L.mx_fail_host, L.mx_fail.p, sizeof(unsigned int), cudaMemcpyDeviceToHost, s));
    RG_CUDA(cudaEventRecord(L.mx_ev, s));
    L.mx_pending = true; L.mx_bs = bs; L.mx_block_id = block_id;
    h->mx_blocks += 1;
    return;
  }
  enqueue_solve_f64(h, L, d, s);
  if (!h->loocv) enqueue_predict(h, L, d, L.cm.p, (int64_t)d.n_aug * d.nC, d.nC, d.nC, s);
}


static void l0_block_dense(rg_ctx* h, const uint8_t* probs, const uint8_t* miss, const double* G64, int64_t n_file, int bs,
                           const int32_t* sample_idx, int ref_first, int block_id) {
  RG_CHECK(n_file > 0, "bad sample count of the genotype file");
  BlockDims d;
  rg_ctx::Lane& L = l0_begin_block(h, bs, block_id, sample_idx, d);
  resolve_lane(h, L);
  const int C = h->C, P = h->P, K = h->K, R = h->R;
  const int64_t Npad = h->Npad;
  cudaStream_t s = L.stream;
  L.last_pred_i8 = 0; L.last_mx_n = 0;

  L.gd.alloc((size_t)h->bs_max * Npad);
  L.mu.alloc(h->rows_p_max);
  L.inv_sd.alloc(h->rows_p_max);
  if (G64) {
    const double* src = G64;
    if (!is_device_pointer(G64)) {
      L.dense_in.alloc((size_t)h->bs_max * n_file * 8);
      copy_to_device(L.dense_in.p, G64, (size_t)bs * n_file * 8, s);
      src = reinterpret_cast<const double*>(L.dense_in.p);
    }
    launch_dense_from_f64(src, n_file, bs, h->file_idx_pad.p, L.gd.p, Npad, s);
  } else {
    const uint8_t *pd = probs, *md = miss;
    if (!is_device_pointer(probs)) {
      L.dense_in.alloc((size_t)h->bs_max * n_file * 3);
      copy_to_device(L.dense_in.p, probs, (size_t)bs * n_file * 2, s);
      pd = L.dense_in.p;
      if (miss) {
        copy_to_device(L.dense_in.p + (size_t)h->bs_max * n_file * 2, miss, (size_t)bs * n_file, s);
        md = L.dense_in.p + (size_t)h->bs_max * n_file * 2;
      }
    }
    launch_dense_from_dosage(pd, md, n_file, bs, h->file_idx_pad.p, ref_first, L.gd.p, Npad, s);
  }
  launch_dense_prepare(L.gd.p, Npad, bs, h->file_idx_pad.p, h->xy.p, h->cpp, C, h->n_analyzed, 1e-6, L.mu.p, L.inv_sd.p,
                       h->err_slot.p, (long long)block_id * h->bs_max, s);
  const int nC = d.nC, nch = h->nchunks;
  const int64_t part_stride = (int64_t)nC * nC;
  L.dpart.alloc((size_t)nch * round_up(h->bs_max, 64) * round_up(h->bs_max, 64));
  L.dpart_y.alloc((size_t)P * nch * h->bs_max);
  launch_l1_gram(L.gd.p, Npad, bs, h->chunks.p, nch, L.dpart.p, part_stride, nC, s);
  for (int p = 0; p < P; ++p)
    launch_l1_xty(L.gd.p, Npad, h->xy.p, h->cpp, C + p, h->chunks.p, nch, L.dpart_y.p + (size_t)p * nch * bs, bs, s);
  ensure_f64_systems(h, L, d, s);
  const int64_t cm_stride = (int64_t)d.n_aug * nC;
  launch_dense_assemble(L.dpart.p, part_stride, nC, L.dpart_y.p, (int64_t)nch * bs, h->fold_chunks.p, K, R, h->lambda.p, bs, nC,
                        P, L.cm.p, cm_stride, h->loocv, s);
  if (h->loocv) launch_dense_loocv_fill(L.gd.p, Npad, bs, nC, L.cm.p, cm_stride, nC + d.Ppad, R, s);
  launch_chol_factor(L.cm.p, cm_stride, nC, d.n_aug, d.nmat, L.inv.p, h->err_slot.p,
                     (long long)(1ll << 40) + (long long)block_id * 1024, s);
  h->launches += 5 + P + chol_num_launches(nC);
  L.part.alloc((size_t)d.ntiles_s * d.Qp * 2);
  L.mean_invsd.alloc((size_t)2 * d.Qp);
  if (h->loocv) {
    enqueue_loocv_predict(h, L, d, s);
    return;
  }
  launch_chol_backsolve(L.cm.p, cm_stride, nC, P, d.nmat, L.inv.p, s);
  launch_dense_predict(L.gd.p, Npad, bs, L.cm.p, cm_stride, nC, nC, R, P, h->tile_fold.p, h->mask.p, h->W_tab.p, d.col0, s);
  const int nparts = launch_l0_colsum(h->W_tab.p, Npad, d.col0, P, d.Q, d.Qp, L.part.p, s);
  launch_l0_standardize(L.part.p, nparts, d.Qp, d.Q, P, h->neff.p, L.mean_invsd.p, h->W_tab.p, Npad, d.col0, h->is_real.p, s);
  h->launches += 6;
}

struct DebugView {
  const void* dev = nullptr;
  std::vector<uint8_t> host;
  size_t bytes = 0;
};

static DebugView dev_view(const void* p, size_t bytes) {
  DebugView v;
  v.dev = p;
  v.bytes = bytes;
  return v;
}

template <class T>
static DebugView host_view(const T* p, size_t count) {
  DebugView v;
  v.host.assign(reinterpret_cast<const uint8_t*>(p), reinterpret_cast<const uint8_t*>(p + count));
  v.bytes = v.host.size();
  return v;
}

static DebugView s2_debug_view(const rg_ctx* h, const std::string& n) {
  if (n == "s2_paths") {
    const int64_t v[8] = {h->s2_tc ? 1 : 0, h->s2_nchunk, h->s2_chunk_len, h->s2_drows, h->nchunks, h->Npad, h->dp, h->bt_dp};
    return host_view(v, 8);
  }
  if (n == "s2_sums") return dev_view(h->s2_sums.p, (size_t)h->s2_sums_rows * 3 * h->dp * 8);
  if (n == "bt_sums") return dev_view(h->bt_sums.p, (size_t)h->bt_sums_rows * 4 * h->bt_sums_dp * 8);
  if (n == "bt_nnz") return dev_view(h->bt_nnz.p, (size_t)h->bt_sums_rows * 8);
  if (n == "bt_n510") return dev_view(h->bt_n510.p, (size_t)h->bt_sums_rows * 8);
  throw Error{"unknown Step-2 debug buffer: " + n};
}

static DebugView l1_debug_view(const rg_ctx* h, const std::string& n) {
  RG_CHECK(h->l1_done, "no level-1 fit on this handle: " + n);
  const int64_t nC = h->l1_nC, P = h->P;
  if (n == "l1_dims") {
    const int64_t v[8] = {h->B, nC, h->R1, h->K, h->l1_nmat, h->l1_n_aug, h->l1_nchunks, h->l1_chunk_len};
    return host_view(v, 8);
  }
  if (n == "l1_chunks") return dev_view(h->l1_chunks.p, (size_t)h->l1_nchunks * sizeof(int4));
  if (n == "l1_beta" && !h->loocv) return dev_view(h->l1_beta.p, (size_t)P * h->K * h->R1 * nC * 8);
  if (n == "l1_sums" && !h->l1_bt) return dev_view(h->l1_sums.p, (size_t)P * (kMaxRidge * 3 + 2) * 8);
  if (n == "l1_bvec" && h->loocv) return dev_view(h->l1_bvec.p, (size_t)P * nC * 8);
  if (n == "l1_hvec" && h->loocv) return dev_view(h->l1_hvec.p, (size_t)P * h->Npad * 8);
  throw Error{"no level-1 debug buffer " + n + " for this fit"};
}

static DebugView l0_debug_view(rg_ctx* h, const std::string& n) {
  RG_CHECK(!h->lanes.empty(), "no level-0 lane: " + n);
  rg_ctx::Lane& L = *h->lanes[h->last_lane];
  const int rp = h->last_rows_p;
  if (n == "gp") return dev_view(L.gp.p, (size_t)rp * (h->Npad / 16) * 4);
  if (n == "z") return dev_view(L.z.p, (size_t)2 * rp * h->Npad);
  if (n == "zz") return dev_view(L.zz.p, (size_t)h->K * 4 * rp * rp * 4);
  if (n == "mu") return dev_view(L.mu.p, (size_t)rp * 8);
  if (n == "inv_sd") return dev_view(L.inv_sd.p, (size_t)rp * 8);
  if (n == "Bv") return dev_view(L.Bv.p, (size_t)rp * h->C * 8);
  if (n == "gty_f") return dev_view(L.gty_f.p, (size_t)h->K * rp * h->P * 8);
  if (n == "rhs") return dev_view(L.rhs.p, (size_t)h->K * rp * h->P * 8);
  if (n == "cm") return dev_view(L.cm.p, (size_t)h->last_nmat * h->last_n_aug * h->last_nC * 8);
  if (n == "mean_invsd") return dev_view(L.mean_invsd.p, (size_t)2 * h->R * h->P * 8);
  if (n == "wraw") return dev_view(L.wraw.p, (size_t)h->P * h->R * h->Npad * 8);
  if (n == "gam" || n == "gmu" || n == "cvec") {
    const size_t Kg = h->loocv ? 1 : h->K, Qp = (size_t)round_up(h->R * h->P, predict_qt());
    const DevBuf<double>& b = n == "gam" ? L.gam : n == "gmu" ? L.gmu : L.cvec;
    return dev_view(b.p, (n == "cvec" ? Kg * Qp * h->C : Kg * rp * Qp) * 8);
  }
  if (n == "cnt_fold") return dev_view(L.cnt_fold.p, (size_t)h->K * rp * 4 * 4);
  if (n == "sum_fold") return dev_view(L.sum_fold.p, (size_t)h->K * rp * 2 * h->cpp * 8);
  if (n == "paths") {
    const int64_t v[3] = {h->stats_tc ? 1 : 0, L.last_pred_i8, L.last_mx_n};
    return host_view(v, 3);
  }
  if (n == "dims") {
    const int64_t v[8] = {h->Npad, rp, h->last_nC, h->last_n_aug, h->last_nmat, h->K, h->cpp, h->nchunks};
    return host_view(v, 8);
  }
  if (n == "gram_path") {
    int64_t v[3] = {0, -1, h->miss_cap};
    if (!L.last_gram_dense) {
      RG_CHECK(L.miss_total.p, "debug buffer not filled yet: gram_path");
      unsigned long long tot = 0;
      RG_CUDA(cudaStreamSynchronize(L.stream));
      RG_CUDA(cudaMemcpy(&tot, L.miss_total.p, sizeof(tot), cudaMemcpyDeviceToHost));
      v[0] = (int64_t)tot <= h->miss_cap ? 1 : 0;
      v[1] = (int64_t)tot;
    }
    return host_view(v, 3);
  }
  if (n == "pad_of") return host_view(h->pad_of.data(), h->N);
  if (n == "zz_ref") {
    RG_CHECK(L.z.p, "debug buffer not filled yet: z");
    const size_t per = (size_t)4 * rp * rp;
    DevBuf<float> ref;
    ref.alloc(per * h->K);
    RG_CUDA(cudaMemsetAsync(ref.p, 0, per * h->K * 4, h->stream));
    for (int f = 0; f < h->K; ++f)
      launch_gram_reference(L.z.p, h->Npad, 2 * rp, (int)h->fold_pad_start[f], (int)(h->fold_pad_start[f] + h->fold_pad_len[f]),
                            ref.p + per * f, 2 * rp, h->stream);
    std::vector<float> v(per * h->K);
    RG_CUDA(cudaMemcpyAsync(v.data(), ref.p, v.size() * 4, cudaMemcpyDeviceToHost, h->stream));
    RG_CUDA(cudaStreamSynchronize(h->stream));
    return host_view(v.data(), v.size());
  }
  throw Error{"unknown debug buffer: " + n};
}

static DebugView debug_view(rg_ctx* h, const std::string& n, int64_t max_bytes) {
  if (n == "pgen_rows") {
    const DevBuf<uint8_t>& r = h->kind == 1 && !h->lanes.empty() ? h->lanes[h->next_lane]->packed_dev : h->pgen_rows;
    RG_CHECK(r.p, "pgen_rows: no rg_pgen_decode has filled it");
    return dev_view(r.p, std::min<size_t>(r.n, (size_t)std::max<int64_t>(max_bytes, 0)));
  }
  if (h->kind == 2) return s2_debug_view(h, n);
  if (n.compare(0, 3, "l1_") == 0) return l1_debug_view(h, n);
  return l0_debug_view(h, n);
}

static int64_t copy_debug_view(const DebugView& v, const std::string& n, void* out, int64_t max_bytes) {
  RG_CHECK(v.dev || !v.host.empty(), "debug buffer not filled yet: " + n);
  RG_CHECK((int64_t)v.bytes <= max_bytes, "buffer too small for " + n + ": it needs " + std::to_string(v.bytes) + " bytes");
  if (v.dev) RG_CUDA(cudaMemcpy(out, v.dev, v.bytes, cudaMemcpyDeviceToHost));
  else memcpy(out, v.host.data(), v.bytes);
  return (int64_t)v.bytes;
}

}

using namespace rg;

extern "C" {

const char* rg_last_error(void) { return rg::g_last_error.c_str(); }
const char* rg_version(void) { return "regenie_b200 0.1 (sm_90a)"; }

int rg_device_count(void) {
  int n = 0;
  if (cudaGetDeviceCount(&n) != cudaSuccess) {
    cudaGetLastError();
    return 0;
  }
  return n;
}

int rg_warmup(int32_t device) {
  RG_API_BEGIN
  require_gpu(device);
  RG_CUDA(cudaSetDevice(device));
  RG_CUDA(cudaFree(nullptr));
  RG_API_END
}

int rg_step1_create(const rg_step1_config* cfg, const double* X, const double* Y, const uint8_t* mask,
                    const uint8_t* in_analysis, const int64_t* fold_sizes, const double* lambda,
                    const double* neff, rg_handle* out) {
  RG_API_BEGIN
  RG_CHECK(cfg && X && Y && mask && in_analysis && lambda && neff && out, "null argument");
  require_gpu(cfg->device);
  RG_CHECK(cfg->n_samples > 0 && cfg->n_cov > 0 && cfg->n_pheno > 0, "bad sizes");
  RG_CHECK(cfg->n_cov <= kMaxCov, "too many covariates for this build");
  RG_CHECK(cfg->loocv || (cfg->n_folds >= 2 && cfg->n_folds <= kMaxFolds), "n_folds out of range");
  RG_CHECK(cfg->n_ridge_l0 >= 1 && cfg->max_block_size >= 1 && cfg->total_blocks >= 1, "bad sizes");
  RG_CUDA(cudaSetDevice(cfg->device));
  std::unique_ptr<rg_ctx> h(new rg_ctx());
  h->kind = 1;
  h->device = cfg->device;
  RG_CUDA(cudaStreamCreateWithFlags(&h->stream, cudaStreamNonBlocking));
  {
    int nl = 8;
    if (const char* q = getenv("CUDA_DEVICE_MAX_CONNECTIONS")) if (atoi(q) >= 16) nl = 12;
    if (const char* e = getenv("RG_B200_LANES")) nl = std::max(1, std::min(32, atoi(e)));
    for (int i = 0; i < nl; ++i) {
      auto l = std::make_unique<rg_ctx::Lane>();
      RG_CUDA(cudaStreamCreateWithFlags(&l->stream, cudaStreamNonBlocking));
      RG_CUDA(cudaEventCreateWithFlags(&l->done, cudaEventDisableTiming));
      h->lanes.push_back(std::move(l));
    }
  }
  h->N = cfg->n_samples; h->C = cfg->n_cov; h->P = cfg->n_pheno;
  h->loocv = cfg->loocv ? 1 : 0;
  h->K = h->loocv ? 1 : cfg->n_folds;
  h->R = cfg->n_ridge_l0; h->R1 = cfg->n_ridge_l1;
  h->bs_max = cfg->max_block_size;
  h->rows_p_max = (int)round_up(h->bs_max, kRowPad);
  h->total_blocks = cfg->total_blocks;
  h->B = (int64_t)h->total_blocks * h->R;
  h->n_analyzed = cfg->n_analyzed;
  if (const char* e = getenv("RG_B200_SOLVER")) h->solver_mixed = std::string(e) == "f64" ? 0 : 1;
  if (const char* e = getenv("RG_B200_MX_TOL")) h->mx_tol = (float)atof(e);
  build_layout(h.get(), X, Y, mask, in_analysis, fold_sizes);
  h->lambda.alloc(h->R);
  h->neff.alloc(h->P);
  RG_CUDA(cudaMemcpy(h->lambda.p, lambda, h->R * 8, cudaMemcpyHostToDevice));
  RG_CUDA(cudaMemcpy(h->neff.p, neff, h->P * 8, cudaMemcpyHostToDevice));
  h->err_slot.alloc(1);
  RG_CUDA(cudaMemset(h->err_slot.p, 0xFF, 8));
  h->W_owned.assign(h->P, 1);
  h->W_host_tab.resize(h->P);
  h->W_host_tab.assign(h->P, nullptr);
  h->W_tab.alloc(h->P);
  h->l1_select.assign(h->P, 1);
  *out = h.release();
  RG_API_END
}

void rg_destroy(rg_handle h) {
  if (!h) return;
  cudaSetDevice(h->device);
  for (void* m : h->W_peer_mapped) cudaIpcCloseMemHandle(m);
  if (h->poll_stream) { cudaStreamSynchronize(h->poll_stream); cudaStreamDestroy(h->poll_stream); }
  if (h->poll_host) cudaFreeHost(h->poll_host);
  for (auto& l : h->lanes) cudaStreamSynchronize(l->stream);
  cudaStreamSynchronize(h->stream);
  rg::flush_timers(h);
  for (auto& l : h->lanes) {
    if (l->mx_ev) cudaEventDestroy(l->mx_ev);
    if (l->h2d_done) cudaEventDestroy(l->h2d_done);
    for (int k = 0; k < 2; ++k) if (l->relayout_done[k]) cudaEventDestroy(l->relayout_done[k]);
    if (l->copy_stream) { cudaStreamSynchronize(l->copy_stream); cudaStreamDestroy(l->copy_stream); }
    if (l->mx_fail_host) cudaFreeHost(l->mx_fail_host);
    cudaEventDestroy(l->done);
    cudaStreamDestroy(l->stream);
  }
  cudaStreamDestroy(h->stream);
  if (h->s2_hd) cudaFreeHost(h->s2_hd);
  if (h->s2_hi) cudaFreeHost(h->s2_hi);
  if (h->s2_copy_stream) { cudaStreamSynchronize(h->s2_copy_stream); cudaStreamDestroy(h->s2_copy_stream); }
  for (int k = 0; k < rg_ctx::kStageSlots; ++k) if (h->s2_stage_ev[k]) cudaEventDestroy(h->s2_stage_ev[k]);
  delete h;
}

int rg_W_export(rg_handle h, void* ipc_handle_64) {
  RG_API_BEGIN
  RG_CHECK(h && h->kind == 1 && ipc_handle_64, "bad argument");
  static_assert(sizeof(cudaIpcMemHandle_t) == 64, "cudaIpcMemHandle_t is 64 bytes");
  RG_CUDA(cudaSetDevice(h->device));
  ensure_W(h);
  cudaIpcMemHandle_t mh;
  RG_CUDA(cudaIpcGetMemHandle(&mh, h->W.p));
  memcpy(ipc_handle_64, &mh, 64);
  RG_API_END
}

int rg_W_set_owned(rg_handle h, const uint8_t* owned) {
  RG_API_BEGIN
  RG_CHECK(h && h->kind == 1 && owned, "bad argument");
  rg::sync_lanes(h);
  RG_CHECK(!h->W.p, "rg_W_set_owned must be called before the first block / export");
  h->W_owned.assign(owned, owned + h->P);
  for (int p = 0; p < h->P; ++p) h->l1_select[p] = owned[p] ? 1 : 0;
  ensure_W(h);
  RG_API_END
}

int rg_W_attach_peer(rg_handle h, const void* ipc_handle_64, const uint8_t* owned_by_peer) {
  RG_API_BEGIN
  RG_CHECK(h && h->kind == 1 && ipc_handle_64 && owned_by_peer, "bad argument");
  rg::sync_lanes(h);
  ensure_W(h);
  cudaIpcMemHandle_t mh;
  memcpy(&mh, ipc_handle_64, 64);
  void* base = nullptr;
  RG_CUDA(cudaIpcOpenMemHandle(&base, mh, cudaIpcMemLazyEnablePeerAccess));
  h->W_peer_mapped.push_back(base);
  size_t slot = 0;
  for (int p = 0; p < h->P; ++p)
    if (owned_by_peer[p]) {
      h->W_host_tab[p] = static_cast<double*>(base) + (slot++) * (size_t)h->Npad * h->B;
      h->l1_select[p] = 0;
    }
  RG_CUDA(cudaMemcpy(h->W_tab.p, h->W_host_tab.data(), h->P * sizeof(double*), cudaMemcpyHostToDevice));
  RG_API_END
}

int rg_W_attach_local(rg_handle h, rg_handle peer, const uint8_t* owned_by_peer) {
  RG_API_BEGIN
  RG_CHECK(h && peer && h != peer && h->kind == 1 && peer->kind == 1 && owned_by_peer, "bad argument");
  RG_CHECK(h->P == peer->P && h->Npad == peer->Npad && h->B == peer->B, "handles describe different problems");
  RG_CUDA(cudaSetDevice(peer->device));
  ensure_W(peer);
  rg::sync_lanes(h);
  ensure_W(h);
  if (h->device != peer->device) {
    int can = 0;
    RG_CUDA(cudaDeviceCanAccessPeer(&can, h->device, peer->device));
    RG_CHECK(can, "no peer access between the two devices");
    const cudaError_t e = cudaDeviceEnablePeerAccess(peer->device, 0);
    if (e == cudaErrorPeerAccessAlreadyEnabled) cudaGetLastError();
    else RG_CUDA(e);
  }
  size_t slot = 0;
  for (int p = 0; p < h->P; ++p)
    if (owned_by_peer[p]) {
      RG_CHECK(peer->W_owned[p], "the peer does not own storage for a phenotype it is said to own");
      h->W_host_tab[p] = peer->W.p + (slot++) * (size_t)h->Npad * h->B;
      h->l1_select[p] = 0;
    }
  RG_CUDA(cudaMemcpy(h->W_tab.p, h->W_host_tab.data(), h->P * sizeof(double*), cudaMemcpyHostToDevice));
  RG_API_END
}

int rg_l1_select(rg_handle h, const uint8_t* sel) {
  RG_API_BEGIN
  RG_CHECK(h && h->kind == 1 && sel, "bad argument");
  h->l1_select.assign(sel, sel + h->P);
  RG_API_END
}

int rg_sync(rg_handle h) {
  RG_API_BEGIN
  RG_CHECK(h, "null handle");
  rg::sync_lanes(h);
  RG_CUDA(cudaStreamSynchronize(h->stream));
  rg::flush_timers(h);
  rg::pgen_check_errors(h);
  RG_API_END
}

int rg_fence(rg_handle h) {
  RG_API_BEGIN
  RG_CHECK(h, "null handle");
  RG_CUDA(cudaSetDevice(h->device));
  if (h->kind == 1) for (auto& l : h->lanes) rg::resolve_lane(h, *l);
  for (auto& l : h->lanes) {
    RG_CUDA(cudaEventRecord(l->done, l->stream));
    RG_CUDA(cudaStreamWaitEvent(h->stream, l->done, 0));
  }
  RG_API_END
}

int rg_l0_block_bed(rg_handle h, const uint8_t* packed, int64_t row_stride, int32_t bs,
                    const int32_t* sample_idx, int32_t ref_first, int32_t block_id) {
  RG_API_BEGIN
  RG_CHECK(h && packed, "null argument");
  l0_block_bed(h, packed, row_stride, bs, sample_idx, ref_first, block_id);
  RG_CUDA(cudaGetLastError());
  RG_API_END
}

int rg_l0_block_dosage_u8(rg_handle h, const uint8_t* probs, const uint8_t* ploidy_missing, int64_t n_file, int32_t bs,
                          const int32_t* sample_idx, int32_t ref_first, int32_t block_id) {
  RG_API_BEGIN
  RG_CHECK(h && probs, "null argument");
  l0_block_dense(h, probs, ploidy_missing, nullptr, n_file, bs, sample_idx, ref_first, block_id);
  RG_CUDA(cudaGetLastError());
  RG_API_END
}

int rg_l0_block_f64(rg_handle h, const double* G, int64_t n_file, int32_t bs, const int32_t* sample_idx, int32_t block_id) {
  RG_API_BEGIN
  RG_CHECK(h && G, "null argument");
  l0_block_dense(h, nullptr, nullptr, G, n_file, bs, sample_idx, 0, block_id);
  RG_CUDA(cudaGetLastError());
  RG_API_END
}

int rg_l0_wait_input(rg_handle h) {
  RG_API_BEGIN
  RG_CHECK(h && h->kind == 1, "not a Step-1 handle");
  RG_CUDA(cudaSetDevice(h->device));
  rg_ctx::Lane& L = *h->lanes[h->last_lane];
  if (L.h2d_recorded) RG_CUDA(cudaEventSynchronize(L.h2d_done));
  RG_API_END
}

int rg_l0_load_W(rg_handle h, int32_t block_id, int32_t ph, const double* in) {
  RG_API_BEGIN
  RG_CHECK(h && in, "null argument");
  RG_CHECK(h->kind == 1 && block_id >= 0 && block_id < h->total_blocks && ph >= 0 && ph < h->P, "bad index");
  RG_CUDA(cudaSetDevice(h->device));
  std::vector<double> tmp((size_t)h->Npad * h->R, 0.0);
  for (int r = 0; r < h->R; ++r)
    for (int64_t s = 0; s < h->N; ++s) tmp[(size_t)r * h->Npad + h->pad_of[s]] = in[(size_t)r * h->N + s];
  ensure_W(h);
  RG_CHECK(h->W_host_tab[ph] != nullptr, "this rank holds no storage for that phenotype (rg_W_set_owned)");
  double* dst = h->W_host_tab[ph] + (size_t)block_id * h->R * h->Npad;
  RG_CUDA(cudaMemcpyAsync(dst, tmp.data(), tmp.size() * 8, cudaMemcpyHostToDevice, h->stream));
  RG_CUDA(cudaStreamSynchronize(h->stream));
  RG_API_END
}

int64_t rg_l0_status(rg_handle h) {
  if (!h) return -1;
  cudaSetDevice(h->device);
  try { rg::sync_lanes(h); } catch (const rg::Error& e) { rg::set_last_error(e.msg); return -1; }
  if (cudaStreamSynchronize(h->stream) != cudaSuccess) {
    rg::set_last_error(std::string("CUDA error: ") + cudaGetErrorString(cudaGetLastError()));
    return -1;
  }
  rg::flush_timers(h);
  try { rg::pgen_check_errors(h); } catch (const rg::Error& e) { rg::set_last_error(e.msg); return (int64_t)1 << 41; }
  unsigned long long v = 0;
  cudaMemcpy(&v, h->err_slot.p, 8, cudaMemcpyDeviceToHost);
  if (v == ~0ull) return 0;
  if (v >= (1ull << 40)) {
    rg::set_last_error("Cholesky pivot not positive (system id " + std::to_string(v - (1ull << 40)) + ")");
    return (int64_t)v;
  }
  rg::set_last_error("SNP has low variance (index " + std::to_string(v - 1) + ")");
  return (int64_t)v;
}

int64_t rg_l0_poll_status(rg_handle h) {
  if (!h || h->kind != 1 || !h->err_slot.p) return -1;
  cudaSetDevice(h->device);
  if (!h->poll_stream && cudaStreamCreateWithFlags(&h->poll_stream, cudaStreamNonBlocking) != cudaSuccess) return -1;
  if (!h->poll_host && cudaHostAlloc((void**)&h->poll_host, 8, cudaHostAllocDefault) != cudaSuccess) return -1;
  if (cudaMemcpyAsync(h->poll_host, h->err_slot.p, 8, cudaMemcpyDeviceToHost, h->poll_stream) != cudaSuccess ||
      cudaStreamSynchronize(h->poll_stream) != cudaSuccess) {
    rg::set_last_error(std::string("CUDA error: ") + cudaGetErrorString(cudaGetLastError()));
    return -1;
  }
  const unsigned long long v = *h->poll_host;
  if (v == ~0ull) return 0;
  if (v >= (1ull << 40)) rg::set_last_error("Cholesky pivot not positive (system id " + std::to_string(v - (1ull << 40)) + ")");
  else rg::set_last_error("SNP has low variance (index " + std::to_string(v - 1) + ")");
  return (int64_t)v;
}

int rg_l0_fetch_W(rg_handle h, int32_t block_id, int32_t ph, double* out) {
  RG_API_BEGIN
  RG_CHECK(h && out, "null argument");
  RG_CHECK(h->kind == 1 && block_id >= 0 && block_id < h->total_blocks && ph >= 0 && ph < h->P, "bad index");
  rg::sync_lanes(h);
  std::vector<double> tmp((size_t)h->Npad * h->R);
  ensure_W(h);
  RG_CHECK(h->W_host_tab[ph] != nullptr, "this rank holds no storage for that phenotype (rg_W_set_owned)");
  const double* src = h->W_host_tab[ph] + (size_t)block_id * h->R * h->Npad;
  RG_CUDA(cudaMemcpyAsync(tmp.data(), src, tmp.size() * 8, cudaMemcpyDeviceToHost, h->stream));
  RG_CUDA(cudaStreamSynchronize(h->stream));
  for (int r = 0; r < h->R; ++r)
    for (int64_t s = 0; s < h->N; ++s) out[(size_t)r * h->N + s] = tmp[(size_t)r * h->Npad + h->pad_of[s]];
  RG_API_END
}

int64_t rg_debug_fetch(rg_handle h, const char* name, void* out, int64_t max_bytes) {
  if (!h || !name || !out) { rg::set_last_error("rg_debug_fetch: null argument"); return -1; }
  cudaSetDevice(h->device);
  try {
    rg::sync_lanes(h);
    cudaStreamSynchronize(h->stream);
    const std::string n(name);
    return rg::copy_debug_view(rg::debug_view(h, n, max_bytes), n, out, max_bytes);
  } catch (const rg::Error& e) {
    rg::set_last_error(e.msg);
    return -1;
  }
}

int rg_l0_solver_stats(rg_handle h, int64_t* mixed_blocks, int64_t* f64_fallbacks) {
  RG_API_BEGIN
  RG_CHECK(h && h->kind == 1, "not a Step-1 handle");
  rg::sync_lanes(h);
  if (mixed_blocks) *mixed_blocks = h->mx_blocks;
  if (f64_fallbacks) *f64_fallbacks = h->mx_fallbacks;
  RG_API_END
}

int rg_dbg_mixed_solve(int32_t device, int32_t n, int32_t K, int32_t R, int32_t P, const double* Af,
                       const double* lambda, const double* b, int32_t steps, double tol, double* x_out,
                       float* X_out, uint32_t* fail_out) {
  RG_API_BEGIN
  RG_CHECK(Af && lambda && b && x_out && fail_out, "null argument");
  rg::require_gpu(device);
  RG_CUDA(cudaSetDevice(device));
  const int Pp = (int)rg::round_up(P, 2), nmat = K * R;
  rg::MixedSolver mx;
  mx.prepare(n, K, R, Pp);
  rg::DevBuf<double> dA, dl, db, dx, dr;
  rg::DevBuf<unsigned int> dfail;
  dA.alloc((size_t)K * n * n); dl.alloc(R); db.alloc((size_t)K * Pp * n); dx.alloc((size_t)nmat * Pp * n); dr.alloc((size_t)nmat * Pp * n);
  dfail.alloc(1);
  RG_CUDA(cudaMemset(db.p, 0, db.n * 8));
  RG_CUDA(cudaMemset(dx.p, 0, dx.n * 8));
  RG_CUDA(cudaMemset(dfail.p, 0, 4));
  RG_CUDA(cudaMemcpy(dA.p, Af, dA.n * 8, cudaMemcpyHostToDevice));
  {
    std::vector<float> pl((size_t)K * n * n);
    for (size_t e = 0; e < pl.size(); ++e) pl[e] = (float)Af[e];
    RG_CUDA(cudaMemcpy(mx.a_planes(), pl.data(), pl.size() * 4, cudaMemcpyHostToDevice));
  }
  RG_CUDA(cudaMemcpy(dl.p, lambda, R * 8, cudaMemcpyHostToDevice));
  for (int f = 0; f < K; ++f)
    RG_CUDA(cudaMemcpy(db.p + (size_t)f * Pp * n, b + (size_t)f * P * n, (size_t)P * n * 8, cudaMemcpyHostToDevice));
  cudaStream_t st;
  RG_CUDA(cudaStreamCreateWithFlags(&st, cudaStreamNonBlocking));
  mx.solve(dA.p, dl.p, db.p, dx.p, dr.p, P, steps, (float)tol, dfail.p, st);
  cudaError_t e = cudaGetLastError();
  if (e == cudaSuccess) e = cudaStreamSynchronize(st);
  cudaStreamDestroy(st);
  RG_CHECK(e == cudaSuccess, std::string("mixed solver kernels failed: ") + cudaGetErrorString(e));
  for (int m = 0; m < nmat; ++m)
    RG_CUDA(cudaMemcpy(x_out + (size_t)m * P * n, dx.p + (size_t)m * Pp * n, (size_t)P * n * 8, cudaMemcpyDeviceToHost));
  if (X_out) RG_CUDA(cudaMemcpy(X_out, mx.debug_planes(2), (size_t)nmat * n * n * 4, cudaMemcpyDeviceToHost));
  RG_CUDA(cudaMemcpy(fail_out, dfail.p, 4, cudaMemcpyDeviceToHost));
  RG_API_END
}

int64_t rg_launch_count(rg_handle h) { return h ? h->launches : 0; }
void* rg_stream(rg_handle h) { return h ? (void*)h->stream : nullptr; }

int rg_set_timing(rg_handle h, int32_t enable) {
  RG_API_BEGIN
  RG_CHECK(h, "null handle");
  h->timing = enable != 0;
  RG_API_END
}

int rg_get_timing(rg_handle h, const char* kernel, double* total_ms, int64_t* launches) {
  RG_API_BEGIN
  RG_CHECK(h && kernel, "null argument");
  rg::sync_lanes(h);
  RG_CUDA(cudaStreamSynchronize(h->stream));
  rg::flush_timers(h);
  auto it = h->timers.find(kernel);
  if (total_ms) *total_ms = it == h->timers.end() ? 0.0 : it->second.first;
  if (launches) *launches = it == h->timers.end() ? 0 : it->second.second;
  RG_API_END
}

int rg_timing_reset(rg_handle h) {
  RG_API_BEGIN
  RG_CHECK(h, "null handle");
  RG_CUDA(cudaStreamSynchronize(h->stream));
  rg::flush_timers(h);
  h->timers.clear();
  RG_API_END
}

}
```

regenie_b200/csrc/wgmma_sm90.cuh:

```cuda
#pragma once
#include <cuda.h>
#include <stdint.h>

namespace rg {
namespace sm90 {

constexpr uint32_t kSpinLimit = 1u << 28;

__device__ __forceinline__ uint32_t smem_u32(const void* p) { return (uint32_t)__cvta_generic_to_shared(p); }
__device__ __forceinline__ void mbar_init(uint32_t bar, uint32_t count) {
  asm volatile("mbarrier.init.shared::cta.b64 [%0], %1;" ::"r"(bar), "r"(count) : "memory");
}
__device__ __forceinline__ void mbar_expect_tx(uint32_t bar, uint32_t bytes) {
  asm volatile("mbarrier.arrive.expect_tx.shared::cta.b64 _, [%0], %1;" ::"r"(bar), "r"(bytes) : "memory");
}
__device__ __forceinline__ void mbar_arrive(uint32_t bar) {
  asm volatile("mbarrier.arrive.shared::cta.b64 _, [%0];" ::"r"(bar) : "memory");
}
__device__ __forceinline__ void mbar_wait(uint32_t bar, uint32_t parity) {
  uint32_t done = 0, spins = 0;
  while (true) {
    asm volatile(
        "{\n\t.reg .pred p;\n\t"
        "mbarrier.try_wait.parity.shared::cta.b64 p, [%1], %2;\n\t"
        "selp.u32 %0, 1, 0, p;\n\t}"
        : "=r"(done) : "r"(bar), "r"(parity) : "memory");
    if (done) break;
    if (++spins > kSpinLimit) __trap();
  }
}
__device__ __forceinline__ void fence_barrier_init() {
  asm volatile("fence.mbarrier_init.release.cluster;" ::: "memory");
  asm volatile("fence.proxy.async.shared::cta;" ::: "memory");
}
__device__ __forceinline__ void prefetch_tmap(const CUtensorMap* tm) {
  asm volatile("prefetch.tensormap [%0];" ::"l"(tm) : "memory");
}
__device__ __forceinline__ void tma_load_2d(uint32_t dst, const CUtensorMap* tm, uint32_t bar, int c0, int c1) {
  asm volatile(
      "cp.async.bulk.tensor.2d.shared::cluster.global.mbarrier::complete_tx::bytes [%0], [%1, {%3, %4}], [%2];"
      ::"r"(dst), "l"(tm), "r"(bar), "r"(c0), "r"(c1) : "memory");
}
__device__ __forceinline__ void tma_load_3d(uint32_t dst, const CUtensorMap* tm, uint32_t bar, int c0, int c1, int c2) {
  asm volatile(
      "cp.async.bulk.tensor.3d.shared::cluster.global.mbarrier::complete_tx::bytes [%0], [%1, {%3, %4, %5}], [%2];"
      ::"r"(dst), "l"(tm), "r"(bar), "r"(c0), "r"(c1), "r"(c2) : "memory");
}
__device__ __forceinline__ void named_sync(int id, int nthreads) {
  asm volatile("bar.sync %0, %1;" ::"r"(id), "r"(nthreads) : "memory");
}

__device__ __forceinline__ uint64_t desc_k128(uint32_t addr) {
  uint64_t d = 0;
  d |= (uint64_t)((addr >> 4) & 0x3FFF);
  d |= (uint64_t)1 << 16;
  d |= (uint64_t)(1024 >> 4) << 32;
  d |= (uint64_t)1 << 62;
  return d;
}

__device__ __forceinline__ void wgmma_fence() { asm volatile("wgmma.fence.sync.aligned;" ::: "memory"); }
__device__ __forceinline__ void wgmma_commit() { asm volatile("wgmma.commit_group.sync.aligned;" ::: "memory"); }
template <int N>
__device__ __forceinline__ void wgmma_wait() { asm volatile("wgmma.wait_group.sync.aligned %0;" ::"n"(N) : "memory"); }
template <typename T, int N>
__device__ __forceinline__ void fence_regs(T (&d)[N]) {
#pragma unroll
  for (int i = 0; i < N; ++i) asm volatile("" : "+r"(reinterpret_cast<uint32_t&>(d[i])) :: "memory");
}


__device__ __forceinline__ void wgmma_s8_n256(int32_t (&d)[128], uint64_t da, uint64_t db) {
  asm volatile(
      "wgmma.mma_async.sync.aligned.m64n256k32.s32.s8.s8 "
      "{%0, %1, %2, %3, %4, %5, %6, %7, %8, %9, %10, %11, %12, %13, %14, %15, %16, %17, %18, %19, %20, %21, %22, %23, %24, %25, %26, %27, %28, %29, %30, %31, %32, %33, %34, %35, %36, %37, %38, %39, %40, %41, %42, %43, %44, %45, %46, %47, %48, %49, %50, %51, %52, %53, %54, %55, %56, %57, %58, %59, %60, %61, %62, %63, %64, %65, %66, %67, %68, %69, %70, %71, %72, %73, %74, %75, %76, %77, %78, %79, %80, %81, %82, %83, %84, %85, %86, %87, %88, %89, %90, %91, %92, %93, %94, %95, %96, %97, %98, %99, %100, %101, %102, %103, %104, %105, %106, %107, %108, %109, %110, %111, %112, %113, %114, %115, %116, %117, %118, %119, %120, %121, %122, %123, %124, %125, %126, %127}, %128, %129, 1;"
      : "+r"(d[0]), "+r"(d[1]), "+r"(d[2]), "+r"(d[3]), "+r"(d[4]), "+r"(d[5]), "+r"(d[6]), "+r"(d[7]), "+r"(d[8]), "+r"(d[9]), "+r"(d[10]), "+r"(d[11]), "+r"(d[12]), "+r"(d[13]), "+r"(d[14]), "+r"(d[15]), "+r"(d[16]), "+r"(d[17]), "+r"(d[18]), "+r"(d[19]), "+r"(d[20]), "+r"(d[21]), "+r"(d[22]), "+r"(d[23]), "+r"(d[24]), "+r"(d[25]), "+r"(d[26]), "+r"(d[27]), "+r"(d[28]), "+r"(d[29]), "+r"(d[30]), "+r"(d[31]), "+r"(d[32]), "+r"(d[33]), "+r"(d[34]), "+r"(d[35]), "+r"(d[36]), "+r"(d[37]), "+r"(d[38]), "+r"(d[39]), "+r"(d[40]), "+r"(d[41]), "+r"(d[42]), "+r"(d[43]), "+r"(d[44]), "+r"(d[45]), "+r"(d[46]), "+r"(d[47]), "+r"(d[48]), "+r"(d[49]), "+r"(d[50]), "+r"(d[51]), "+r"(d[52]), "+r"(d[53]), "+r"(d[54]), "+r"(d[55]), "+r"(d[56]), "+r"(d[57]), "+r"(d[58]), "+r"(d[59]), "+r"(d[60]), "+r"(d[61]), "+r"(d[62]), "+r"(d[63]), "+r"(d[64]), "+r"(d[65]), "+r"(d[66]), "+r"(d[67]), "+r"(d[68]), "+r"(d[69]), "+r"(d[70]), "+r"(d[71]), "+r"(d[72]), "+r"(d[73]), "+r"(d[74]), "+r"(d[75]), "+r"(d[76]), "+r"(d[77]), "+r"(d[78]), "+r"(d[79]), "+r"(d[80]), "+r"(d[81]), "+r"(d[82]), "+r"(d[83]), "+r"(d[84]), "+r"(d[85]), "+r"(d[86]), "+r"(d[87]), "+r"(d[88]), "+r"(d[89]), "+r"(d[90]), "+r"(d[91]), "+r"(d[92]), "+r"(d[93]), "+r"(d[94]), "+r"(d[95]), "+r"(d[96]), "+r"(d[97]), "+r"(d[98]), "+r"(d[99]), "+r"(d[100]), "+r"(d[101]), "+r"(d[102]), "+r"(d[103]), "+r"(d[104]), "+r"(d[105]), "+r"(d[106]), "+r"(d[107]), "+r"(d[108]), "+r"(d[109]), "+r"(d[110]), "+r"(d[111]), "+r"(d[112]), "+r"(d[113]), "+r"(d[114]), "+r"(d[115]), "+r"(d[116]), "+r"(d[117]), "+r"(d[118]), "+r"(d[119]), "+r"(d[120]), "+r"(d[121]), "+r"(d[122]), "+r"(d[123]), "+r"(d[124]), "+r"(d[125]), "+r"(d[126]), "+r"(d[127])
      : "l"(da), "l"(db));
}
__device__ __forceinline__ void wgmma_s8_n128(int32_t (&d)[64], uint64_t da, uint64_t db) {
  asm volatile(
      "wgmma.mma_async.sync.aligned.m64n128k32.s32.s8.s8 "
      "{%0, %1, %2, %3, %4, %5, %6, %7, %8, %9, %10, %11, %12, %13, %14, %15, %16, %17, %18, %19, %20, %21, %22, %23, %24, %25, %26, %27, %28, %29, %30, %31, %32, %33, %34, %35, %36, %37, %38, %39, %40, %41, %42, %43, %44, %45, %46, %47, %48, %49, %50, %51, %52, %53, %54, %55, %56, %57, %58, %59, %60, %61, %62, %63}, %64, %65, 1;"
      : "+r"(d[0]), "+r"(d[1]), "+r"(d[2]), "+r"(d[3]), "+r"(d[4]), "+r"(d[5]), "+r"(d[6]), "+r"(d[7]), "+r"(d[8]), "+r"(d[9]), "+r"(d[10]), "+r"(d[11]), "+r"(d[12]), "+r"(d[13]), "+r"(d[14]), "+r"(d[15]), "+r"(d[16]), "+r"(d[17]), "+r"(d[18]), "+r"(d[19]), "+r"(d[20]), "+r"(d[21]), "+r"(d[22]), "+r"(d[23]), "+r"(d[24]), "+r"(d[25]), "+r"(d[26]), "+r"(d[27]), "+r"(d[28]), "+r"(d[29]), "+r"(d[30]), "+r"(d[31]), "+r"(d[32]), "+r"(d[33]), "+r"(d[34]), "+r"(d[35]), "+r"(d[36]), "+r"(d[37]), "+r"(d[38]), "+r"(d[39]), "+r"(d[40]), "+r"(d[41]), "+r"(d[42]), "+r"(d[43]), "+r"(d[44]), "+r"(d[45]), "+r"(d[46]), "+r"(d[47]), "+r"(d[48]), "+r"(d[49]), "+r"(d[50]), "+r"(d[51]), "+r"(d[52]), "+r"(d[53]), "+r"(d[54]), "+r"(d[55]), "+r"(d[56]), "+r"(d[57]), "+r"(d[58]), "+r"(d[59]), "+r"(d[60]), "+r"(d[61]), "+r"(d[62]), "+r"(d[63])
      : "l"(da), "l"(db));
}
__device__ __forceinline__ void wgmma_tf32_n128(float (&d)[64], uint64_t da, uint64_t db) {
  asm volatile(
      "wgmma.mma_async.sync.aligned.m64n128k8.f32.tf32.tf32 "
      "{%0, %1, %2, %3, %4, %5, %6, %7, %8, %9, %10, %11, %12, %13, %14, %15, %16, %17, %18, %19, %20, %21, %22, %23, %24, %25, %26, %27, %28, %29, %30, %31, %32, %33, %34, %35, %36, %37, %38, %39, %40, %41, %42, %43, %44, %45, %46, %47, %48, %49, %50, %51, %52, %53, %54, %55, %56, %57, %58, %59, %60, %61, %62, %63}, %64, %65, 1, 1, 1;"
      : "+f"(d[0]), "+f"(d[1]), "+f"(d[2]), "+f"(d[3]), "+f"(d[4]), "+f"(d[5]), "+f"(d[6]), "+f"(d[7]), "+f"(d[8]), "+f"(d[9]), "+f"(d[10]), "+f"(d[11]), "+f"(d[12]), "+f"(d[13]), "+f"(d[14]), "+f"(d[15]), "+f"(d[16]), "+f"(d[17]), "+f"(d[18]), "+f"(d[19]), "+f"(d[20]), "+f"(d[21]), "+f"(d[22]), "+f"(d[23]), "+f"(d[24]), "+f"(d[25]), "+f"(d[26]), "+f"(d[27]), "+f"(d[28]), "+f"(d[29]), "+f"(d[30]), "+f"(d[31]), "+f"(d[32]), "+f"(d[33]), "+f"(d[34]), "+f"(d[35]), "+f"(d[36]), "+f"(d[37]), "+f"(d[38]), "+f"(d[39]), "+f"(d[40]), "+f"(d[41]), "+f"(d[42]), "+f"(d[43]), "+f"(d[44]), "+f"(d[45]), "+f"(d[46]), "+f"(d[47]), "+f"(d[48]), "+f"(d[49]), "+f"(d[50]), "+f"(d[51]), "+f"(d[52]), "+f"(d[53]), "+f"(d[54]), "+f"(d[55]), "+f"(d[56]), "+f"(d[57]), "+f"(d[58]), "+f"(d[59]), "+f"(d[60]), "+f"(d[61]), "+f"(d[62]), "+f"(d[63])
      : "l"(da), "l"(db));
}
__device__ __forceinline__ void wgmma_tf32_n128_nega(float (&d)[64], uint64_t da, uint64_t db) {
  asm volatile(
      "wgmma.mma_async.sync.aligned.m64n128k8.f32.tf32.tf32 "
      "{%0, %1, %2, %3, %4, %5, %6, %7, %8, %9, %10, %11, %12, %13, %14, %15, %16, %17, %18, %19, %20, %21, %22, %23, %24, %25, %26, %27, %28, %29, %30, %31, %32, %33, %34, %35, %36, %37, %38, %39, %40, %41, %42, %43, %44, %45, %46, %47, %48, %49, %50, %51, %52, %53, %54, %55, %56, %57, %58, %59, %60, %61, %62, %63}, %64, %65, 1, -1, 1;"
      : "+f"(d[0]), "+f"(d[1]), "+f"(d[2]), "+f"(d[3]), "+f"(d[4]), "+f"(d[5]), "+f"(d[6]), "+f"(d[7]), "+f"(d[8]), "+f"(d[9]), "+f"(d[10]), "+f"(d[11]), "+f"(d[12]), "+f"(d[13]), "+f"(d[14]), "+f"(d[15]), "+f"(d[16]), "+f"(d[17]), "+f"(d[18]), "+f"(d[19]), "+f"(d[20]), "+f"(d[21]), "+f"(d[22]), "+f"(d[23]), "+f"(d[24]), "+f"(d[25]), "+f"(d[26]), "+f"(d[27]), "+f"(d[28]), "+f"(d[29]), "+f"(d[30]), "+f"(d[31]), "+f"(d[32]), "+f"(d[33]), "+f"(d[34]), "+f"(d[35]), "+f"(d[36]), "+f"(d[37]), "+f"(d[38]), "+f"(d[39]), "+f"(d[40]), "+f"(d[41]), "+f"(d[42]), "+f"(d[43]), "+f"(d[44]), "+f"(d[45]), "+f"(d[46]), "+f"(d[47]), "+f"(d[48]), "+f"(d[49]), "+f"(d[50]), "+f"(d[51]), "+f"(d[52]), "+f"(d[53]), "+f"(d[54]), "+f"(d[55]), "+f"(d[56]), "+f"(d[57]), "+f"(d[58]), "+f"(d[59]), "+f"(d[60]), "+f"(d[61]), "+f"(d[62]), "+f"(d[63])
      : "l"(da), "l"(db));
}
__device__ __forceinline__ void wgmma_s8_rs_n256(int32_t (&d)[128], const uint32_t (&a)[4], uint64_t db) {
  asm volatile(
      "wgmma.mma_async.sync.aligned.m64n256k32.s32.s8.s8 "
      "{%0, %1, %2, %3, %4, %5, %6, %7, %8, %9, %10, %11, %12, %13, %14, %15, %16, %17, %18, %19, %20, %21, %22, %23, %24, %25, %26, %27, %28, %29, %30, %31, %32, %33, %34, %35, %36, %37, %38, %39, %40, %41, %42, %43, %44, %45, %46, %47, %48, %49, %50, %51, %52, %53, %54, %55, %56, %57, %58, %59, %60, %61, %62, %63, %64, %65, %66, %67, %68, %69, %70, %71, %72, %73, %74, %75, %76, %77, %78, %79, %80, %81, %82, %83, %84, %85, %86, %87, %88, %89, %90, %91, %92, %93, %94, %95, %96, %97, %98, %99, %100, %101, %102, %103, %104, %105, %106, %107, %108, %109, %110, %111, %112, %113, %114, %115, %116, %117, %118, %119, %120, %121, %122, %123, %124, %125, %126, %127}, {%128, %129, %130, %131}, %132, 1;"
      : "+r"(d[0]), "+r"(d[1]), "+r"(d[2]), "+r"(d[3]), "+r"(d[4]), "+r"(d[5]), "+r"(d[6]), "+r"(d[7]), "+r"(d[8]), "+r"(d[9]), "+r"(d[10]), "+r"(d[11]), "+r"(d[12]), "+r"(d[13]), "+r"(d[14]), "+r"(d[15]), "+r"(d[16]), "+r"(d[17]), "+r"(d[18]), "+r"(d[19]), "+r"(d[20]), "+r"(d[21]), "+r"(d[22]), "+r"(d[23]), "+r"(d[24]), "+r"(d[25]), "+r"(d[26]), "+r"(d[27]), "+r"(d[28]), "+r"(d[29]), "+r"(d[30]), "+r"(d[31]), "+r"(d[32]), "+r"(d[33]), "+r"(d[34]), "+r"(d[35]), "+r"(d[36]), "+r"(d[37]), "+r"(d[38]), "+r"(d[39]), "+r"(d[40]), "+r"(d[41]), "+r"(d[42]), "+r"(d[43]), "+r"(d[44]), "+r"(d[45]), "+r"(d[46]), "+r"(d[47]), "+r"(d[48]), "+r"(d[49]), "+r"(d[50]), "+r"(d[51]), "+r"(d[52]), "+r"(d[53]), "+r"(d[54]), "+r"(d[55]), "+r"(d[56]), "+r"(d[57]), "+r"(d[58]), "+r"(d[59]), "+r"(d[60]), "+r"(d[61]), "+r"(d[62]), "+r"(d[63]), "+r"(d[64]), "+r"(d[65]), "+r"(d[66]), "+r"(d[67]), "+r"(d[68]), "+r"(d[69]), "+r"(d[70]), "+r"(d[71]), "+r"(d[72]), "+r"(d[73]), "+r"(d[74]), "+r"(d[75]), "+r"(d[76]), "+r"(d[77]), "+r"(d[78]), "+r"(d[79]), "+r"(d[80]), "+r"(d[81]), "+r"(d[82]), "+r"(d[83]), "+r"(d[84]), "+r"(d[85]), "+r"(d[86]), "+r"(d[87]), "+r"(d[88]), "+r"(d[89]), "+r"(d[90]), "+r"(d[91]), "+r"(d[92]), "+r"(d[93]), "+r"(d[94]), "+r"(d[95]), "+r"(d[96]), "+r"(d[97]), "+r"(d[98]), "+r"(d[99]), "+r"(d[100]), "+r"(d[101]), "+r"(d[102]), "+r"(d[103]), "+r"(d[104]), "+r"(d[105]), "+r"(d[106]), "+r"(d[107]), "+r"(d[108]), "+r"(d[109]), "+r"(d[110]), "+r"(d[111]), "+r"(d[112]), "+r"(d[113]), "+r"(d[114]), "+r"(d[115]), "+r"(d[116]), "+r"(d[117]), "+r"(d[118]), "+r"(d[119]), "+r"(d[120]), "+r"(d[121]), "+r"(d[122]), "+r"(d[123]), "+r"(d[124]), "+r"(d[125]), "+r"(d[126]), "+r"(d[127])
      : "r"(a[0]), "r"(a[1]), "r"(a[2]), "r"(a[3]), "l"(db));
}

}
}
```

Measured before the change: 930,600.

## Fuse 2-bit genotype expansion into the int8 Gram WGMMA kernel

Removes the separate kernel that expanded packed 2-bit genotypes into a 2×rows int8 Z matrix in global memory. The Gram kernel now TMA-loads the packed words directly. A operands are expanded in registers and fed to register-sourced WGMMA, and B operands are expanded into a swizzled shared buffer that is triple-buffered and published through proxy fences and named barriers. This avoids the large Z write and re-read plus one launch, at the cost of extra ALU work and synchronisation inside the matmul mainloop.

```diff
diff --git a/regenie_b200/csrc/bed_kernels.cu b/regenie_b200/csrc/bed_kernels.cu
--- a/regenie_b200/csrc/bed_kernels.cu
+++ b/regenie_b200/csrc/bed_kernels.cu
@@ -48,31 +48,6 @@
   gp[(int64_t)row * words_per_row + w] = out;
 }
 
-__device__ __forceinline__ uint32_t spread_sel(uint32_t b) {
-  return (b & 0x3u) | ((b & 0xCu) << 2) | ((b & 0x30u) << 4) | ((b & 0xC0u) << 6);
-}
-
-__global__ void bed_expand_fp8_kernel(const uint32_t* __restrict__ gp, int64_t words_per_row,
-                                      int rows_p, uint8_t* __restrict__ z, int64_t npad) {
-  const int64_t w = blockIdx.x * (int64_t)blockDim.x + threadIdx.x;
-  const int row = blockIdx.y;
-  if (w >= words_per_row) return;
-  const uint32_t word = __ldg(gp + (int64_t)row * words_per_row + w);
-  const uint32_t kLutG = 0x00100800u;
-  const uint32_t kLutM = 0x08000000u;
-  uint4 g, m;
-  uint32_t* gv = reinterpret_cast<uint32_t*>(&g);
-  uint32_t* mv = reinterpret_cast<uint32_t*>(&m);
-#pragma unroll
-  for (int k = 0; k < 4; ++k) {
-    const uint32_t sel = spread_sel((word >> (8 * k)) & 0xFFu);
-    gv[k] = __byte_perm(kLutG, 0, sel);
-    mv[k] = __byte_perm(kLutM, 0, sel);
-  }
-  *reinterpret_cast<uint4*>(z + (int64_t)row * npad + w * 16) = g;
-  *reinterpret_cast<uint4*>(z + (int64_t)(rows_p + row) * npad + w * 16) = m;
-}
-
 void launch_bed_relayout(const uint8_t* packed, int64_t row_stride, int bs, int rows_p,
                          const int32_t* file_idx_pad, const int32_t* word_base, const uint32_t* word_keep, int ref_first,
                          uint32_t* gp, int64_t npad,
@@ -82,10 +57,4 @@
   bed_relayout_kernel<<<grid, 256, 0, s>>>(packed, row_stride, bs, file_idx_pad, word_base, word_keep, ref_first, gp, wpr);
 }
 
-void launch_bed_expand_fp8(const uint32_t* gp, int rows_p, uint8_t* z, int64_t npad, cudaStream_t s) {
-  const int64_t wpr = npad / 16;
-  dim3 grid((unsigned)ceil_div(wpr, 256), rows_p);
-  bed_expand_fp8_kernel<<<grid, 256, 0, s>>>(gp, wpr, rows_p, z, npad);
 }
-
-}
diff --git a/regenie_b200/csrc/context.cuh b/regenie_b200/csrc/context.cuh
--- a/regenie_b200/csrc/context.cuh
+++ b/regenie_b200/csrc/context.cuh
@@ -55,7 +55,6 @@
     int packed_flip = 0;
     rg::DevBuf<uint8_t> pgen_in;
     rg::DevBuf<uint32_t> gp;
-    rg::DevBuf<uint8_t> z;
     rg::DevBuf<float> zz;
     rg::DevBuf<unsigned long long> miss_total;
     rg::DevBuf<int2> miss_seg;
@@ -68,7 +67,6 @@
     rg::DevBuf<double> cm;
     rg::DevBuf<double> inv;
     rg::DevBuf<double> gam, gmu, cvec, part, mean_invsd;
-    std::map<int, CUtensorMap> tmaps;
     rg::DevBuf<uint8_t> dig;
     rg::DevBuf<double> wraw;
     rg::DevBuf<double*> wraw_tab;
diff --git a/regenie_b200/csrc/gram_wgmma.cu b/regenie_b200/csrc/gram_wgmma.cu
--- a/regenie_b200/csrc/gram_wgmma.cu
+++ b/regenie_b200/csrc/gram_wgmma.cu
@@ -11,29 +11,63 @@
 constexpr int BK = 128;
 constexpr int STAGES = 4;
 constexpr int A_BYTES = BM * BK;
+constexpr int GROW = BK / 16 * 4;
+constexpr int G_BYTES = 128 * GROW;
+constexpr int XBUF = 3;
 constexpr int NTHREADS = 288;
-
-}
-
-template <int BN>
+constexpr uint32_t kLutG0 = 0x00100800u;
+constexpr uint32_t kLutMiss = 0x08000000u;
+
+template <int BN, bool A2, bool B2>
+struct GramLayout {
+  static constexpr int NST = B2 ? 6 : STAGES;
+  static constexpr int A_ST = A2 ? G_BYTES : A_BYTES;
+  static constexpr int B_ST = B2 ? 2 * G_BYTES : BN * BK;
+  static constexpr int X_BYTES = B2 ? XBUF * BN * BK : 0;
+  static constexpr int RING = NST * (A_ST + B_ST);
+  static constexpr size_t SMEM = (size_t)X_BYTES + RING + 1024 + 128;
+};
+
+__device__ __forceinline__ uint32_t code_nibbles(uint32_t n) {
+  n = (n | (n << 4)) & 0x0F0F0F0Fu;
+  return (n | (n << 2)) & 0x33333333u;
+}
+__device__ __forceinline__ void plane_pair(uint32_t x, uint32_t y, uint32_t psel, uint32_t lut, uint32_t& px,
+                                           uint32_t& py) {
+  const uint32_t n = code_nibbles(__byte_perm(x, y, psel) & 0x00FF00FFu);
+  px = __byte_perm(lut, 0, n);
+  py = __byte_perm(lut, 0, n >> 16);
+}
+__device__ __forceinline__ uint4 plane_chunk(uint32_t w, uint32_t lut) {
+  const uint32_t a = code_nibbles(__byte_perm(w, 0, 0x4140)), b = code_nibbles(__byte_perm(w, 0, 0x4342));
+  return make_uint4(__byte_perm(lut, 0, a), __byte_perm(lut, 0, a >> 16), __byte_perm(lut, 0, b),
+                    __byte_perm(lut, 0, b >> 16));
+}
+__device__ __forceinline__ int gp_row(int zrow, int rows_p) { return zrow < rows_p ? zrow : zrow - rows_p; }
+
+}
+
+template <int BN, bool A2, bool B2>
 __global__ void __launch_bounds__(NTHREADS, 1)
-gram_s8_wgmma_kernel(const __grid_constant__ CUtensorMap tmZ, const __grid_constant__ CUtensorMap tmB,
+gram_s8_wgmma_kernel(const __grid_constant__ CUtensorMap tmA, const __grid_constant__ CUtensorMap tmB,
                       const int2* __restrict__ tiles,
                       const int2* __restrict__ fold_k, float* __restrict__ out, int ldo,
                       int64_t fold_stride, float out_scale, const unsigned long long* __restrict__ miss_total,
-                      unsigned long long miss_cap, int miss_tile0) {
-  constexpr int B_BYTES = BN * BK;
-  constexpr int STAGE_BYTES = A_BYTES + B_BYTES;
+                      unsigned long long miss_cap, int miss_tile0, int rows_p) {
+  static_assert(!B2 || (A2 && BN == 256), "2-bit B rows only with 2-bit A rows, in 128 x 256 tiles");
+  using Lo = GramLayout<BN, A2, B2>;
+  constexpr int NST = Lo::NST;
   constexpr int NACC = BN / 2;
   extern __shared__ uint8_t smem_raw[];
   const uint32_t raw = smem_u32(smem_raw);
   const uint32_t base = (raw + 1023u) & ~1023u;
   uint8_t* gen_base = smem_raw + (base - raw);
-  const uint32_t sA = base;
-  const uint32_t sB = base + STAGES * A_BYTES;
-  uint64_t* bars = reinterpret_cast<uint64_t*>(gen_base + STAGES * STAGE_BYTES);
+  const uint32_t sX = base;
+  const uint32_t sB = A2 ? base + Lo::X_BYTES : base + NST * A_BYTES;
+  const uint32_t sA = A2 ? sB + NST * Lo::B_ST : base;
+  uint64_t* bars = reinterpret_cast<uint64_t*>(gen_base + Lo::X_BYTES + Lo::RING);
   const uint32_t full_bar = smem_u32(bars);
-  const uint32_t empty_bar = smem_u32(bars + STAGES);
+  const uint32_t empty_bar = smem_u32(bars + NST);
 
   const int warp = __shfl_sync(0xffffffffu, threadIdx.x >> 5, 0), lane = threadIdx.x & 31;
   const int2 tile = tiles[blockIdx.x];
@@ -42,12 +76,12 @@
   const int nkb = fk.y;
 
   if (warp == 8 && lane == 0) {
-    for (int s = 0; s < STAGES; ++s) {
+    for (int s = 0; s < NST; ++s) {
       mbar_init(full_bar + 8 * s, 1);
       mbar_init(empty_bar + 8 * s, 2);
     }
     fence_barrier_init();
-    prefetch_tmap(&tmZ);
+    prefetch_tmap(&tmA);
     prefetch_tmap(&tmB);
   }
   __syncthreads();
@@ -55,14 +89,21 @@
   if (warp == 8) {
     if (lane == 0) {
       for (int kb = 0; kb < nkb; ++kb) {
-        const int s = kb % STAGES;
-        const uint32_t ph = (kb / STAGES) & 1;
+        const int s = kb % NST;
+        const uint32_t ph = (kb / NST) & 1;
+        const uint32_t fb = full_bar + 8 * s;
         mbar_wait(empty_bar + 8 * s, ph ^ 1);
-        mbar_expect_tx(full_bar + 8 * s, STAGE_BYTES);
+        mbar_expect_tx(fb, Lo::A_ST + Lo::B_ST);
         const int kc = (fk.x + kb) * BK;
-        tma_load_2d(sA + s * A_BYTES, &tmZ, full_bar + 8 * s, kc, tile.x * BM);
-        tma_load_2d(sB + s * B_BYTES, &tmB, full_bar + 8 * s, kc, tile.y * BN);
-        if (BN == 256) tma_load_2d(sB + s * B_BYTES + A_BYTES, &tmB, full_bar + 8 * s, kc, tile.y * BN + 128);
+        if constexpr (A2) tma_load_2d(sA + s * Lo::A_ST, &tmA, fb, kc / 16, gp_row(tile.x * BM, rows_p));
+        else tma_load_2d(sA + s * A_BYTES, &tmA, fb, kc, tile.x * BM);
+        if constexpr (B2) {
+          tma_load_2d(sB + s * Lo::B_ST, &tmB, fb, kc / 16, gp_row(tile.y * BN, rows_p));
+          tma_load_2d(sB + s * Lo::B_ST + G_BYTES, &tmB, fb, kc / 16, gp_row(tile.y * BN + 128, rows_p));
+        } else {
+          tma_load_2d(sB + s * Lo::B_ST, &tmB, fb, kc, tile.y * BN);
+          if (BN == 256) tma_load_2d(sB + s * Lo::B_ST + A_BYTES, &tmB, fb, kc, tile.y * BN + 128);
+        }
       }
     }
     return;
@@ -73,21 +114,86 @@
 #pragma unroll
   for (int i = 0; i < NACC; ++i) acc[i] = 0;
   fence_regs(acc);
-  for (int kb = 0; kb < nkb; ++kb) {
-    const int s = kb % STAGES;
-    const uint32_t ph = (kb / STAGES) & 1;
-    mbar_wait(full_bar + 8 * s, ph);
-    const uint64_t da = desc_k128(sA + s * A_BYTES + wg * (64 * BK));
-    const uint64_t db = desc_k128(sB + s * B_BYTES);
-    wgmma_fence();
-#pragma unroll
-    for (int k = 0; k < BK / 32; ++k) {
-      if constexpr (BN == 256) wgmma_s8_n256(acc, da + (uint64_t)(2 * k), db + (uint64_t)(2 * k));
-      else wgmma_s8_n128(acc, da + (uint64_t)(2 * k), db + (uint64_t)(2 * k));
-    }
-    wgmma_commit();
-    wgmma_wait<1>();
-    if (kb > 0 && (warp & 3) == 0 && lane == 0) mbar_arrive(empty_bar + 8 * ((kb - 1) % STAGES));
+  if constexpr (!A2) {
+    for (int kb = 0; kb < nkb; ++kb) {
+      const int s = kb % NST;
+      const uint32_t ph = (kb / NST) & 1;
+      mbar_wait(full_bar + 8 * s, ph);
+      const uint64_t da = desc_k128(sA + s * A_BYTES + wg * (64 * BK));
+      const uint64_t db = desc_k128(sB + s * Lo::B_ST);
+      wgmma_fence();
+#pragma unroll
+      for (int k = 0; k < BK / 32; ++k) {
+        if constexpr (BN == 256) wgmma_s8_n256(acc, da + (uint64_t)(2 * k), db + (uint64_t)(2 * k));
+        else wgmma_s8_n128(acc, da + (uint64_t)(2 * k), db + (uint64_t)(2 * k));
+      }
+      wgmma_commit();
+      wgmma_wait<1>();
+      if (kb > 0 && (warp & 3) == 0 && lane == 0) mbar_arrive(empty_bar + 8 * ((kb - 1) % NST));
+    }
+  } else {
+    const int w = warp & 3, t4 = lane & 3;
+    const uint32_t psel = (uint32_t)t4 | ((uint32_t)(4 + t4) << 8);
+    const uint32_t lut_a = tile.x * BM >= rows_p ? kLutMiss : kLutG0;
+    const uint8_t* gA = gen_base + (sA - base) + (64 * wg + 16 * w + (lane >> 2)) * GROW;
+    auto build = [&](int s, int kk, uint32_t (&af)[4]) {
+      const uint8_t* p = gA + s * Lo::A_ST + 8 * kk;
+      const uint2 v0 = *reinterpret_cast<const uint2*>(p);
+      const uint2 v1 = *reinterpret_cast<const uint2*>(p + 8 * GROW);
+      plane_pair(v0.x, v0.y, psel, lut_a, af[0], af[2]);
+      plane_pair(v1.x, v1.y, psel, lut_a, af[1], af[3]);
+    };
+    const int ct = threadIdx.x;
+    const uint32_t lut_b0 = tile.y * BN >= rows_p ? kLutMiss : kLutG0;
+    const uint32_t lut_b1 = tile.y * BN + 128 >= rows_p ? kLutMiss : kLutG0;
+    const uint8_t* gB = gen_base + (sB - base) + 4 * ct;
+    uint8_t* gX = gen_base + (ct >> 3) * 128 + ((((ct & 7) ^ (ct >> 3)) & 7) << 4);
+    auto expand = [&](int s, int xb, int i) {
+      const uint32_t v = *reinterpret_cast<const uint32_t*>(gB + s * Lo::B_ST + 1024 * i);
+      *reinterpret_cast<uint4*>(gX + xb * (BN * BK) + 4096 * i) = plane_chunk(v, i < 4 ? lut_b0 : lut_b1);
+    };
+    auto publish = [&]() {
+      asm volatile("fence.proxy.async.shared::cta;" ::: "memory");
+      named_sync(1, 256);
+    };
+    uint32_t afr[2][4];
+    mbar_wait(full_bar, 0);
+    if constexpr (B2) {
+#pragma unroll
+      for (int i = 0; i < 8; ++i) expand(0, 0, i);
+      publish();
+    }
+    build(0, 0, afr[0]);
+    for (int kb = 0; kb < nkb; ++kb) {
+      const int s = kb % NST, s1 = (kb + 1) % NST;
+      const bool more = kb + 1 < nkb;
+      const uint64_t db = desc_k128(B2 ? sX + (kb % XBUF) * (BN * BK) : sB + s * Lo::B_ST);
+#pragma unroll
+      for (int kk = 0; kk < BK / 32; ++kk) {
+        wgmma_fence();
+        if constexpr (BN == 256) wgmma_s8_rs_n256(acc, afr[kk & 1], db + (uint64_t)(2 * kk));
+        else wgmma_s8_rs_n128(acc, afr[kk & 1], db + (uint64_t)(2 * kk));
+        wgmma_commit();
+        wgmma_wait<1>();
+        if (kk == 0 && kb > 0 && w == 0 && lane == 0) mbar_arrive(empty_bar + 8 * ((kb - 1) % NST));
+        if constexpr (B2) {
+          if (more) {
+            if (kk == 0) mbar_wait(full_bar + 8 * s1, ((kb + 1) / NST) & 1);
+            expand(s1, (kb + 1) % XBUF, 2 * kk);
+            expand(s1, (kb + 1) % XBUF, 2 * kk + 1);
+          }
+        }
+        if (kk + 1 < BK / 32) {
+          build(s, kk + 1, afr[(kk + 1) & 1]);
+        } else if (more) {
+          if constexpr (!B2) mbar_wait(full_bar + 8 * s1, ((kb + 1) / NST) & 1);
+          build(s1, 0, afr[0]);
+        }
+      }
+      if constexpr (B2) {
+        if (more) publish();
+      }
+    }
   }
   wgmma_wait<0>();
   fence_regs(acc);
@@ -103,17 +209,20 @@
   }
 }
 
-__global__ void gram_reference_kernel(const uint8_t* __restrict__ z, int64_t npad, int rows2, int k0, int k1,
-                                      float* __restrict__ out, int ldo) {
+__global__ void gram_reference_kernel(const uint32_t* __restrict__ gp, int64_t words_per_row, int rows_p, int k0,
+                                      int k1, float* __restrict__ out, int ldo) {
   const int j = blockIdx.x * blockDim.x + threadIdx.x;
   const int i = blockIdx.y;
-  if (j >= rows2 || j > i) return;
-  const uint8_t* zi = z + (int64_t)i * npad;
-  const uint8_t* zj = z + (int64_t)j * npad;
+  if (j >= 2 * rows_p || j > i) return;
+  const uint32_t* gi = gp + (int64_t)(i % rows_p) * words_per_row;
+  const uint32_t* gj = gp + (int64_t)(j % rows_p) * words_per_row;
+  const bool mi = i >= rows_p, mj = j >= rows_p;
   int acc = 0;
   for (int t = k0; t < k1; ++t) {
-    const int a = zi[t] >> 3;
-    const int b = zj[t] >> 3;
+    const int ci = (gi[t >> 4] >> (2 * (t & 15))) & 3;
+    const int cj = (gj[t >> 4] >> (2 * (t & 15))) & 3;
+    const int a = mi ? ci == 3 : (ci == 3 ? 0 : ci);
+    const int b = mj ? cj == 3 : (cj == 3 ? 0 : cj);
     acc += a * b;
   }
   out[(int64_t)i * ldo + j] = (float)acc;
@@ -146,36 +255,54 @@
   RG_CHECK(r == CUDA_SUCCESS, "cuTensorMapEncodeTiled failed (" + std::to_string((int)r) + ")");
 }
 
-size_t gram_smem_bytes(int bn) {
-  return (size_t)STAGES * (A_BYTES + bn * BK) + 1024 + 128;
-}
-
 void gram_tile_list(int rows2, std::vector<int2>& tiles) {
   tiles.clear();
   for (int nj = 0; nj < rows2 / 256; ++nj)
     for (int mi = 2 * nj; mi < rows2 / BM; ++mi) tiles.push_back(make_int2(mi, nj));
 }
 
+template <int BN, bool A2, bool B2>
+static void launch_gram(const CUtensorMap& tmA, const CUtensorMap& tmB, const int2* tiles, int ntiles,
+                        const int2* fold_k, int K, float* out, int ldo, int64_t fold_stride, float out_scale,
+                        cudaStream_t s, const unsigned long long* miss_total, int64_t miss_cap, int miss_tile0,
+                        int rows_p) {
+  const void* fn = reinterpret_cast<const void*>(gram_s8_wgmma_kernel<BN, A2, B2>);
+  const size_t smem = GramLayout<BN, A2, B2>::SMEM;
+  ensure_dyn_smem(fn, smem);
+  gram_s8_wgmma_kernel<BN, A2, B2><<<dim3(ntiles, K), NTHREADS, smem, s>>>(
+      tmA, tmB, tiles, fold_k, out, ldo, fold_stride, out_scale, miss_total, miss_cap, miss_tile0, rows_p);
+}
+
 void launch_gram_wgmma(const CUtensorMap& tm, const CUtensorMap& tmB, const int2* tiles, int ntiles, const int2* fold_k, int K,
-                         float* out, int ldo, int64_t fold_stride, float out_scale, cudaStream_t s, int bn,
-                         const unsigned long long* miss_total, int64_t miss_cap, int miss_tile0) {
+                         float* out, int ldo, int64_t fold_stride, float out_scale, cudaStream_t s, int bn) {
   RG_CHECK(bn == 256 || bn == 128, "gram tiles are 128 x 256 or 128 x 128");
-  dim3 grid(ntiles, K);
-  if (bn == 256) {
-    ensure_dyn_smem(reinterpret_cast<const void*>(gram_s8_wgmma_kernel<256>), gram_smem_bytes(256));
-    gram_s8_wgmma_kernel<256><<<grid, NTHREADS, gram_smem_bytes(256), s>>>(tm, tmB, tiles, fold_k, out, ldo, fold_stride, out_scale,
-                                                                                     miss_total, miss_cap, miss_tile0);
+  if (bn == 256) launch_gram<256, false, false>(tm, tmB, tiles, ntiles, fold_k, K, out, ldo, fold_stride, out_scale, s, nullptr, 0, 0, 0);
+  else launch_gram<128, false, false>(tm, tmB, tiles, ntiles, fold_k, K, out, ldo, fold_stride, out_scale, s, nullptr, 0, 0, 0);
+}
+
+void launch_gram_gp(const CUtensorMap& tmG, const CUtensorMap* tmD, int rows_p, const int2* tiles, int ntiles,
+                    const int2* fold_k, int K, float* out, int ldo, int64_t fold_stride, float out_scale, cudaStream_t s,
+                    int bn, const unsigned long long* miss_total, int64_t miss_cap, int miss_tile0) {
+  RG_CHECK(rows_p % 128 == 0, "gram tiles: rows_p is a multiple of 128");
+  if (!tmD) {
+    RG_CHECK(bn == 256, "Z Z^T tiles are 128 x 256");
+    launch_gram<256, true, true>(tmG, tmG, tiles, ntiles, fold_k, K, out, ldo, fold_stride, out_scale, s, miss_total,
+                                 miss_cap, miss_tile0, rows_p);
   } else {
-    ensure_dyn_smem(reinterpret_cast<const void*>(gram_s8_wgmma_kernel<128>), gram_smem_bytes(128));
-    gram_s8_wgmma_kernel<128><<<grid, NTHREADS, gram_smem_bytes(128), s>>>(tm, tmB, tiles, fold_k, out, ldo, fold_stride, out_scale,
-                                                                                     miss_total, miss_cap, miss_tile0);
-  }
-}
-
-void launch_gram_reference(const uint8_t* z, int64_t npad, int rows2, int k0, int k1, float* out, int ldo,
+    RG_CHECK(bn == 256 || bn == 128, "gram tiles are 128 x 256 or 128 x 128");
+    if (bn == 256)
+      launch_gram<256, true, false>(tmG, *tmD, tiles, ntiles, fold_k, K, out, ldo, fold_stride, out_scale, s,
+                                    miss_total, miss_cap, miss_tile0, rows_p);
+    else
+      launch_gram<128, true, false>(tmG, *tmD, tiles, ntiles, fold_k, K, out, ldo, fold_stride, out_scale, s, miss_total,
+                                    miss_cap, miss_tile0, rows_p);
+  }
+}
+
+void launch_gram_reference(const uint32_t* gp, int64_t npad, int rows_p, int k0, int k1, float* out, int ldo,
                            cudaStream_t s) {
-  dim3 grid((unsigned)ceil_div(rows2, 128), rows2);
-  gram_reference_kernel<<<grid, 128, 0, s>>>(z, npad, rows2, k0, k1, out, ldo);
-}
-
-}
+  dim3 grid((unsigned)ceil_div(2 * rows_p, 128), 2 * rows_p);
+  gram_reference_kernel<<<grid, 128, 0, s>>>(gp, npad / 16, rows_p, k0, k1, out, ldo);
+}
+
+}
diff --git a/regenie_b200/csrc/kernels.cuh b/regenie_b200/csrc/kernels.cuh
--- a/regenie_b200/csrc/kernels.cuh
+++ b/regenie_b200/csrc/kernels.cuh
@@ -15,7 +15,6 @@
                          const int32_t* file_idx_pad, const int32_t* word_base, const uint32_t* word_keep, int ref_first,
                          uint32_t* gp, int64_t npad,
                          cudaStream_t s);
-void launch_bed_expand_fp8(const uint32_t* gp, int rows_p, uint8_t* z, int64_t npad, cudaStream_t s);
 
 struct SnpFinalizeArgs {
   int bs, rows_p, C, P, K, cpp, loocv;
@@ -55,7 +54,6 @@
 void launch_l0_assemble(const AssembleArgs& a, const double* rhs, int P, int Ppad, int nmat, cudaStream_t s);
 
 void make_gram_tensor_map(CUtensorMap* tm, const uint8_t* z, int64_t npad, int rows2);
-size_t gram_smem_bytes(int bn = 256);
 constexpr int kStatQ = 14;
 constexpr int kStatOnesRow = 126;
 void launch_l0_xy_digits(const double* xy, int cpp, int ncol, int64_t npad, const uint8_t* is_real, double* scale,
@@ -65,8 +63,11 @@
                             int32_t* cnt_fold, double* sum_fold, cudaStream_t s);
 void gram_tile_list(int rows2, std::vector<int2>& tiles);
 void launch_gram_wgmma(const CUtensorMap& tm, const CUtensorMap& tmB, const int2* tiles, int ntiles, const int2* fold_k, int K,
-                         float* out, int ldo, int64_t fold_stride, float out_scale, cudaStream_t s, int bn = 256,
-                         const unsigned long long* miss_total = nullptr, int64_t miss_cap = 0, int miss_tile0 = 0);
+                         float* out, int ldo, int64_t fold_stride, float out_scale, cudaStream_t s, int bn = 256);
+void launch_gram_gp(const CUtensorMap& tmG, const CUtensorMap* tmD, int rows_p, const int2* tiles, int ntiles,
+                    const int2* fold_k, int K, float* out, int ldo, int64_t fold_stride, float out_scale, cudaStream_t s,
+                    int bn = 256, const unsigned long long* miss_total = nullptr, int64_t miss_cap = 0,
+                    int miss_tile0 = 0);
 constexpr float kZScaleGram = 1.f / 64;
 constexpr float kZScaleStat = 1.f / 8;
 constexpr double kMissSparseRate = 0.015;
@@ -76,7 +77,7 @@
                            uint32_t* gt, cudaStream_t s);
 void launch_miss_sparse(const uint32_t* gt, int rows_p, const int2* seg, const int32_t* list, int K,
                         const unsigned long long* total, int64_t cap, float* zz, int64_t fold_stride, cudaStream_t s);
-void launch_gram_reference(const uint8_t* z, int64_t npad, int rows2, int k0, int k1, float* out, int ldo,
+void launch_gram_reference(const uint32_t* gp, int64_t npad, int rows_p, int k0, int k1, float* out, int ldo,
                            cudaStream_t s);
 
 void launch_chol_factor(double* cm, int64_t stride, int nC, int n_aug, int batch, double* inv,
diff --git a/regenie_b200/csrc/rg_api.cu b/regenie_b200/csrc/rg_api.cu
--- a/regenie_b200/csrc/rg_api.cu
+++ b/regenie_b200/csrc/rg_api.cu
@@ -375,6 +375,16 @@
   }
 }
 
+static const CUtensorMap& gp_map(const rg_ctx* h, rg_ctx::Lane& L, int rows_p) {
+  auto it = L.gmaps.find(rows_p);
+  if (it == L.gmaps.end()) {
+    CUtensorMap tm;
+    make_gp_tensor_map(&tm, L.gp.p, h->Npad / 16, rows_p);
+    it = L.gmaps.emplace(rows_p, tm).first;
+  }
+  return it->second;
+}
+
 static void enqueue_predict(rg_ctx* h, rg_ctx::Lane& L, const BlockDims& d, const double* xsrc, int64_t xstride, int xld,
                             int xrow0, cudaStream_t s) {
   const int C = h->C, P = h->P, K = h->K, R = h->R;
@@ -415,18 +425,13 @@
       make_byte_tensor_map(&tm, L.dig.p, 2 * d.rows_p, (int64_t)K * ngroups * drows_per_group);
       L.dmaps[d.rows_p] = tm;
     }
-    if (!L.gmaps.count(d.rows_p)) {
-      CUtensorMap tm;
-      make_gp_tensor_map(&tm, L.gp.p, Npad / 16, d.rows_p);
-      L.gmaps[d.rows_p] = tm;
-    }
     launch_l0_coef_i8(xsrc, xstride, xld, xrow0, R, P, d.Q, d.Qp, d.bs, d.rows_p, K, L.mu.p, L.inv_sd.p, L.Bv.p, C,
                       L.gam.p, L.gmu.p, L.cvec.p, L.dscale.p, L.dig.p, ngroups, s);
     PredictTcArgs ta;
     ta.rows_p = d.rows_p; ta.C = C; ta.P = P; ta.Q = d.Q; ta.Qp = d.Qp; ta.cpp = h->cpp; ta.col0 = 0; ta.ngroups = ngroups;
     ta.npad = Npad; ta.tile_fold = h->tile_fold.p; ta.scale = L.dscale.p; ta.cvec = L.cvec.p;
     ta.xy = h->xy.p; ta.mask = h->mask.p; ta.W = L.wraw_tab.p; ta.part = L.part.p;
-    launch_l0_predict_i8(L.gmaps[d.rows_p], L.dmaps[d.rows_p], ta, d.ntiles_s, s);
+    launch_l0_predict_i8(gp_map(h, L, d.rows_p), L.dmaps[d.rows_p], ta, d.ntiles_s, s);
     h->launches += 2;
   }
   launch_l0_standardize(L.part.p, d.ntiles_s, d.Qp, d.Q, P, h->neff.p, L.mean_invsd.p, h->W_tab.p, Npad, d.col0,
@@ -523,7 +528,6 @@
   resolve_lane(h, L);
 
   L.gp.alloc((size_t)h->rows_p_max * (Npad / 16));
-  L.z.alloc((size_t)2 * h->rows_p_max * Npad);
   L.zz.alloc((size_t)K * 4 * h->rows_p_max * h->rows_p_max);
   L.cnt_part.alloc((size_t)h->nchunks * h->rows_p_max * 4);
   L.sum_part.alloc((size_t)h->nchunks * h->rows_p_max * 2 * h->cpp);
@@ -552,11 +556,7 @@
       L.relayout_recorded[staged] = true;
     }
   }
-  {
-    ScopedTimer t(h, "bed_expand", s);
-    launch_bed_expand_fp8(L.gp.p, rows_p, L.z.p, Npad, s);
-  }
-  h->launches += 2;
+  h->launches += 1;
 
   auto snp_finalize = [&]() {
     SnpFinalizeArgs a;
@@ -580,18 +580,13 @@
   }
 
   {
-    if (!L.tmaps.count(rows_p)) {
-      CUtensorMap tm;
-      make_gram_tensor_map(&tm, L.z.p, Npad, 2 * rows_p);
-      L.tmaps[rows_p] = tm;
-    }
     const rg_ctx::TileList& tl =
         cached_tiles(h->tile_lists, rows_p, [&](std::vector<int2>& tiles) { gram_tile_list(2 * rows_p, tiles); });
     const int64_t zz_stride = (int64_t)4 * rows_p * rows_p;
     ScopedTimer t(h, "gram_wgmma", s);
     if (h->gram_dense) {
-      launch_gram_wgmma(L.tmaps[rows_p], L.tmaps[rows_p], tl.buf.p, tl.count, h->fold_k.p, K,
-                        L.zz.p, 2 * rows_p, zz_stride, kZScaleGram, s);
+      launch_gram_gp(gp_map(h, L, rows_p), nullptr, rows_p, tl.buf.p, tl.count, h->fold_k.p, K,
+                     L.zz.p, 2 * rows_p, zz_stride, kZScaleGram, s);
       h->launches += 1;
     } else {
       L.miss_total.alloc(1);
@@ -600,8 +595,8 @@
       L.gt.alloc((size_t)Npad * (h->rows_p_max / 16));
       launch_miss_list(L.gp.p, Npad, rows_p, h->fold_k.p, K, L.miss_total.p, h->miss_cap, L.miss_seg.p, L.miss_list.p, s);
       launch_miss_transpose(L.gp.p, Npad, rows_p, L.miss_total.p, h->miss_cap, L.gt.p, s);
-      launch_gram_wgmma(L.tmaps[rows_p], L.tmaps[rows_p], tl.buf.p, tl.count, h->fold_k.p, K,
-                        L.zz.p, 2 * rows_p, zz_stride, kZScaleGram, s, 256, L.miss_total.p, h->miss_cap, rows_p / 128);
+      launch_gram_gp(gp_map(h, L, rows_p), nullptr, rows_p, tl.buf.p, tl.count, h->fold_k.p, K,
+                     L.zz.p, 2 * rows_p, zz_stride, kZScaleGram, s, 256, L.miss_total.p, h->miss_cap, rows_p / 128);
       launch_miss_sparse(L.gt.p, rows_p, L.miss_seg.p, L.miss_list.p, K, L.miss_total.p, h->miss_cap, L.zz.p, zz_stride, s);
       h->launches += 5;
     }
@@ -616,8 +611,8 @@
     });
     L.tstat.alloc((size_t)K * 2 * h->rows_p_max * h->stat_drows);
     const int64_t tfs = (int64_t)2 * rows_p * h->stat_drows;
-    launch_gram_wgmma(L.tmaps[rows_p], h->tmD, tl.buf.p, tl.count, h->fold_k.p,
-                      K, L.tstat.p, h->stat_drows, tfs, kZScaleStat, s, stat_bn);
+    launch_gram_gp(gp_map(h, L, rows_p), &h->tmD, rows_p, tl.buf.p, tl.count, h->fold_k.p,
+                   K, L.tstat.p, h->stat_drows, tfs, kZScaleStat, s, stat_bn);
     launch_l0_stats_finish(L.tstat.p, h->stat_drows, tfs, L.zz.p, 2 * rows_p, (int64_t)4 * rows_p * rows_p, rows_p,
                            h->cpp, C + P, K, h->xy_scale.p, L.cnt_fold.p, L.sum_fold.p, s);
     snp_finalize();
@@ -758,8 +753,9 @@
   rg_ctx::Lane& L = *h->lanes[h->last_lane];
   const int rp = h->last_rows_p;
   if (n == "gp") return dev_view(L.gp.p, (size_t)rp * (h->Npad / 16) * 4);
-  if (n == "z") return dev_view(L.z.p, (size_t)2 * rp * h->Npad);
   if (n == "zz") return dev_view(L.zz.p, (size_t)h->K * 4 * rp * rp * 4);
+  if (n == "tstat" && h->stats_tc) return dev_view(L.tstat.p, (size_t)h->K * 2 * rp * h->stat_drows * 4);
+  if (n == "xyD" && h->stats_tc) return dev_view(h->xyD.p, (size_t)h->stat_drows * h->Npad);
   if (n == "mu") return dev_view(L.mu.p, (size_t)rp * 8);
   if (n == "inv_sd") return dev_view(L.inv_sd.p, (size_t)rp * 8);
   if (n == "Bv") return dev_view(L.Bv.p, (size_t)rp * h->C * 8);
@@ -797,13 +793,13 @@
   }
   if (n == "pad_of") return host_view(h->pad_of.data(), h->N);
   if (n == "zz_ref") {
-    RG_CHECK(L.z.p, "debug buffer not filled yet: z");
+    RG_CHECK(L.gp.p, "debug buffer not filled yet: gp");
     const size_t per = (size_t)4 * rp * rp;
     DevBuf<float> ref;
     ref.alloc(per * h->K);
     RG_CUDA(cudaMemsetAsync(ref.p, 0, per * h->K * 4, h->stream));
     for (int f = 0; f < h->K; ++f)
-      launch_gram_reference(L.z.p, h->Npad, 2 * rp, (int)h->fold_pad_start[f], (int)(h->fold_pad_start[f] + h->fold_pad_len[f]),
+      launch_gram_reference(L.gp.p, h->Npad, rp, (int)h->fold_pad_start[f], (int)(h->fold_pad_start[f] + h->fold_pad_len[f]),
                             ref.p + per * f, 2 * rp, h->stream);
     std::vector<float> v(per * h->K);
     RG_CUDA(cudaMemcpyAsync(v.data(), ref.p, v.size() * 4, cudaMemcpyDeviceToHost, h->stream));
diff --git a/regenie_b200/csrc/wgmma_sm90.cuh b/regenie_b200/csrc/wgmma_sm90.cuh
--- a/regenie_b200/csrc/wgmma_sm90.cuh
+++ b/regenie_b200/csrc/wgmma_sm90.cuh
@@ -105,6 +105,13 @@
       : "+r"(d[0]), "+r"(d[1]), "+r"(d[2]), "+r"(d[3]), "+r"(d[4]), "+r"(d[5]), "+r"(d[6]), "+r"(d[7]), "+r"(d[8]), "+r"(d[9]), "+r"(d[10]), "+r"(d[11]), "+r"(d[12]), "+r"(d[13]), "+r"(d[14]), "+r"(d[15]), "+r"(d[16]), "+r"(d[17]), "+r"(d[18]), "+r"(d[19]), "+r"(d[20]), "+r"(d[21]), "+r"(d[22]), "+r"(d[23]), "+r"(d[24]), "+r"(d[25]), "+r"(d[26]), "+r"(d[27]), "+r"(d[28]), "+r"(d[29]), "+r"(d[30]), "+r"(d[31]), "+r"(d[32]), "+r"(d[33]), "+r"(d[34]), "+r"(d[35]), "+r"(d[36]), "+r"(d[37]), "+r"(d[38]), "+r"(d[39]), "+r"(d[40]), "+r"(d[41]), "+r"(d[42]), "+r"(d[43]), "+r"(d[44]), "+r"(d[45]), "+r"(d[46]), "+r"(d[47]), "+r"(d[48]), "+r"(d[49]), "+r"(d[50]), "+r"(d[51]), "+r"(d[52]), "+r"(d[53]), "+r"(d[54]), "+r"(d[55]), "+r"(d[56]), "+r"(d[57]), "+r"(d[58]), "+r"(d[59]), "+r"(d[60]), "+r"(d[61]), "+r"(d[62]), "+r"(d[63]), "+r"(d[64]), "+r"(d[65]), "+r"(d[66]), "+r"(d[67]), "+r"(d[68]), "+r"(d[69]), "+r"(d[70]), "+r"(d[71]), "+r"(d[72]), "+r"(d[73]), "+r"(d[74]), "+r"(d[75]), "+r"(d[76]), "+r"(d[77]), "+r"(d[78]), "+r"(d[79]), "+r"(d[80]), "+r"(d[81]), "+r"(d[82]), "+r"(d[83]), "+r"(d[84]), "+r"(d[85]), "+r"(d[86]), "+r"(d[87]), "+r"(d[88]), "+r"(d[89]), "+r"(d[90]), "+r"(d[91]), "+r"(d[92]), "+r"(d[93]), "+r"(d[94]), "+r"(d[95]), "+r"(d[96]), "+r"(d[97]), "+r"(d[98]), "+r"(d[99]), "+r"(d[100]), "+r"(d[101]), "+r"(d[102]), "+r"(d[103]), "+r"(d[104]), "+r"(d[105]), "+r"(d[106]), "+r"(d[107]), "+r"(d[108]), "+r"(d[109]), "+r"(d[110]), "+r"(d[111]), "+r"(d[112]), "+r"(d[113]), "+r"(d[114]), "+r"(d[115]), "+r"(d[116]), "+r"(d[117]), "+r"(d[118]), "+r"(d[119]), "+r"(d[120]), "+r"(d[121]), "+r"(d[122]), "+r"(d[123]), "+r"(d[124]), "+r"(d[125]), "+r"(d[126]), "+r"(d[127])
       : "r"(a[0]), "r"(a[1]), "r"(a[2]), "r"(a[3]), "l"(db));
 }
+__device__ __forceinline__ void wgmma_s8_rs_n128(int32_t (&d)[64], const uint32_t (&a)[4], uint64_t db) {
+  asm volatile(
+      "wgmma.mma_async.sync.aligned.m64n128k32.s32.s8.s8 "
+      "{%0, %1, %2, %3, %4, %5, %6, %7, %8, %9, %10, %11, %12, %13, %14, %15, %16, %17, %18, %19, %20, %21, %22, %23, %24, %25, %26, %27, %28, %29, %30, %31, %32, %33, %34, %35, %36, %37, %38, %39, %40, %41, %42, %43, %44, %45, %46, %47, %48, %49, %50, %51, %52, %53, %54, %55, %56, %57, %58, %59, %60, %61, %62, %63}, {%64, %65, %66, %67}, %68, 1;"
+      : "+r"(d[0]), "+r"(d[1]), "+r"(d[2]), "+r"(d[3]), "+r"(d[4]), "+r"(d[5]), "+r"(d[6]), "+r"(d[7]), "+r"(d[8]), "+r"(d[9]), "+r"(d[10]), "+r"(d[11]), "+r"(d[12]), "+r"(d[13]), "+r"(d[14]), "+r"(d[15]), "+r"(d[16]), "+r"(d[17]), "+r"(d[18]), "+r"(d[19]), "+r"(d[20]), "+r"(d[21]), "+r"(d[22]), "+r"(d[23]), "+r"(d[24]), "+r"(d[25]), "+r"(d[26]), "+r"(d[27]), "+r"(d[28]), "+r"(d[29]), "+r"(d[30]), "+r"(d[31]), "+r"(d[32]), "+r"(d[33]), "+r"(d[34]), "+r"(d[35]), "+r"(d[36]), "+r"(d[37]), "+r"(d[38]), "+r"(d[39]), "+r"(d[40]), "+r"(d[41]), "+r"(d[42]), "+r"(d[43]), "+r"(d[44]), "+r"(d[45]), "+r"(d[46]), "+r"(d[47]), "+r"(d[48]), "+r"(d[49]), "+r"(d[50]), "+r"(d[51]), "+r"(d[52]), "+r"(d[53]), "+r"(d[54]), "+r"(d[55]), "+r"(d[56]), "+r"(d[57]), "+r"(d[58]), "+r"(d[59]), "+r"(d[60]), "+r"(d[61]), "+r"(d[62]), "+r"(d[63])
+      : "r"(a[0]), "r"(a[1]), "r"(a[2]), "r"(a[3]), "l"(db));
+}
 
 }
 }
```

New measurement: 972,000, median of 6. 1.04x the previous value.
